# arihantb2/direct_lidar_odometry

Hardware: AMD Instinct MI355X
Metric: gicp_iterations_per_sec (higher is better)
Workload: dtype f64

## Files before the change

__graft_entry__.py:

```python
import os
import sys

ROOT = os.path.dirname(os.path.abspath(__file__))
if ROOT not in sys.path:
    sys.path.insert(0, ROOT)


def build() -> None:
    from direct_lidar_odometry_amd import build as b
    lib = b.build()
    assert os.path.exists(lib)
    import direct_lidar_odometry_amd
    from direct_lidar_odometry_amd import nano_gicp
    L = nano_gicp.load_library()
    missing = [s for s in nano_gicp.EXPORTS if not hasattr(L, s)]
    if missing:
        raise RuntimeError(f"libngicp_hip.so lacks {missing}")
    from oracle import oracle as orc
    orc.build(ref=os.path.isdir("/root/reference/include"))


def smoke() -> None:
    import numpy as np
    from direct_lidar_odometry_amd import build as b
    b.build()
    from direct_lidar_odometry_amd import clouds
    from direct_lidar_odometry_amd.nano_gicp import NanoGICP
    from oracle import oracle as orc

    w = clouds.scan_to_scan(10_000)
    g = NanoGICP(device=0)
    o = orc.OracleGICP()
    for e in (g, o):
        e.setMaxCorrespondenceDistance(1.0)
        e.setInputSource(w.source)
        e.setInputTarget(w.target)
    g.align()
    o.align()
    dt, dr = clouds.pose_error(g.getFinalTransformation(), o.getFinalTransformation())
    s = g.stats()
    print(f"smoke: HIP vs oracle pose diff {dt:.2e} m / {dr:.2e} rad; iterations {g.nr_iterations_ + 1} vs {o.nr_iterations + 1}; "
          f"align {s['align_ms']:.3f} ms; error vs ground truth {clouds.pose_error(g.getFinalTransformation(), w.gt)}")
    if not (dt <= 1e-4 and dr <= 1e-4 and g.nr_iterations_ == o.nr_iterations and g.converged_ == o.converged):
        raise AssertionError("HIP NanoGICP disagrees with the CPU oracle")


if __name__ == "__main__":
    build()
    if "--smoke" in sys.argv:
        smoke()
```

direct_lidar_odometry_amd/build.py:

```python
from __future__ import annotations

import os
import shutil
import subprocess
import sys

HERE = os.path.dirname(os.path.abspath(__file__))
CSRC = os.path.join(HERE, "csrc")
LIB = os.path.join(HERE, "libngicp_hip.so")
SOURCES = ["ngicp_api.hip", "ngicp_filters.hip"]
PUBLIC_HEADER = os.path.normpath(os.path.join(HERE, "..", "include", "ngicp.h"))
DEP_SUFFIXES = (".h", ".inc", ".hip")
FLAGS = ["--offload-arch=gfx950", "-O3", "-std=c++17", "-ffp-contract=off", "-fPIC", "-shared", "-Wall", "-Wno-unused-function"]


def hipcc() -> str:
    for cand in (os.environ.get("HIPCC"), shutil.which("hipcc"), "/opt/rocm/bin/hipcc"):
        if cand and os.path.exists(cand):
            return cand
    raise RuntimeError("hipcc not found")


def dependencies() -> list[str]:
    found = [os.path.join(d, f) for d, _, files in os.walk(CSRC) for f in files if f.endswith(DEP_SUFFIXES)]
    return sorted(found) + [PUBLIC_HEADER, os.path.abspath(__file__)]


def needs_build() -> bool:
    if not os.path.exists(LIB):
        return True
    t = os.path.getmtime(LIB)
    return any(os.path.getmtime(d) > t for d in dependencies())


def build(force: bool = False, verbose: bool = False, extra_flags: list[str] | None = None) -> str:
    if not force and not needs_build():
        return LIB
    tmp = f"{LIB}.{os.getpid()}.tmp"
    cmd = [hipcc(), *FLAGS, *(extra_flags or []), *[os.path.join(CSRC, s) for s in SOURCES], "-o", tmp]
    if verbose:
        print(" ".join(cmd), flush=True)
    res = subprocess.run(cmd, capture_output=True, text=True)
    if res.returncode != 0:
        sys.stderr.write(res.stdout + res.stderr)
        raise RuntimeError("hipcc failed")
    if verbose and res.stderr:
        sys.stderr.write(res.stderr)
    os.replace(tmp, LIB)
    return LIB


if __name__ == "__main__":
    print(build(force="--force" in sys.argv, verbose=True))
```

direct_lidar_odometry_amd/csrc/ngicp_align.h:

```cpp
#pragma once

namespace {

std::mutex& persist_mutex(int device) {
  static std::mutex m[64];
  return m[(unsigned)device % 64u];
}

route::Facts route_facts(const ngicp* h, route::Caller caller, int nblocks = 1) {
  route::Facts f;
  f.caller = caller;
  f.persist = h->persist;
  f.robust = h->robust_kind != NGICP_ROBUST_NONE;
  f.prior = h->prior_set;
  f.iterating = h->p.max_iter > 0;
  f.nblocks = nblocks;
  f.pass_slots = h->pass_slots;
  f.persist_slots = h->persist_slots;
  f.max_passes = max_passes(h->p);
  return f;
}
void refuse_for(const ngicp* h, route::Entry e) {
  const std::string why = route::entry_refusal(e, h->voxel_res > 0.0, h->robust_kind != NGICP_ROBUST_NONE, h->prior_set);
  if (!why.empty()) throw ArgError{NGICP_ERR_ARG, why};
}
void refuse_route(const ngicp* h, route::Caller caller, const char* entry) {
  const std::string why = route::refusal(route::switches(), h->sw, route_facts(h, caller), entry);
  if (!why.empty()) throw ArgError{NGICP_ERR_ARG, why};
}
route::Variant pass_variant(const ngicp* h, route::Caller caller, int nblocks) {
  return route::choose_route(route::switches(), h->sw, route_facts(h, caller, nblocks)).variant;
}
void fill_robust(const ngicp* h, int& kind, double& c, double& c2) {
  kind = h->robust_kind;
  c = h->robust_width;
  c2 = h->robust_width * h->robust_width;
}

void launch_pass(ngicp* h, const PassArgs& a, const route::Variant& v, int nblocks, hipStream_t s, hipEvent_t start = nullptr, hipEvent_t stop = nullptr) {
  using K = void (*)(PassArgs);
  const bool four = v.waves == 4;
  K kernel = nullptr;
  PassArgs b = a;
  unsigned grid = (unsigned)nblocks;
  switch (v.family) {
    case route::Family::Staged: {
      int need = kStGrowMax;
      if (h->p.max_corr_dist < 1e30) need = (int)std::ceil(h->p.max_corr_dist / (double)a.grid.h);
      b.stage_grow = std::max(1, std::min(kStGrowMax, need));
      kernel = four ? K(k_gicp_pass_st<4>) : K(k_gicp_pass_st<3>);
      break;
    }
    case route::Family::Queue:
      grid = (unsigned)std::min(nblocks, h->queue_slots[four]);
      kernel = four ? K(k_gicp_queue<2, 4>) : K(k_gicp_queue<2, 3>);
      break;
    case route::Family::Walks:
      if (v.fused) kernel = four ? K(k_gicp_pass<2, 4, true>) : K(k_gicp_pass<2, 3, true>);
      else if (v.robust) kernel = four ? K(k_gicp_pass<2, 4, false, true>) : K(k_gicp_pass<2, 3, false, true>);
      else kernel = four ? K(k_gicp_pass<2, 4>) : K(k_gicp_pass<2, 3>);
      break;
  }
  hipExtLaunchKernelGGL(kernel, dim3(grid), dim3(256), 0, s, start, stop, 0, b);
}

struct LoopCtx {
  PassArgs pa;
  SolveArgs sa;
  int nblocks;
};

void prepare_loop(ngicp* h, LoopCtx& c, bool own_buffers = true, bool with_target = true) {
  ensure_slot_ready(h, h->src, "source");
  if (with_target) ensure_slot_ready(h, h->tgt, "target");
  if (h->src_covs.n != h->src.dev->n) compute_covs(h, h->src, h->src_covs, "source");
  if (with_target && h->tgt_covs.n != h->tgt.dev->n) compute_covs(h, h->tgt, h->tgt_covs, "target");
  DeviceCloud& S = *h->src.dev;
  const size_t n = S.n;
  const int nblocks = std::max(1, (S.n_batches + 3) / 4);
  const int max_rows = max_trace_rows(h->p);
  if (own_buffers) {
    for (int i = 0; i < 2; ++i) {
      h->tpt[i].ensure(n * sizeof(float4));
      h->mahal[i].ensure(n * 6 * sizeof(double));
    }
    h->partials.ensure((size_t)kNumSlots * nblocks * sizeof(double));
    h->grp_order.ensure((size_t)nblocks * sizeof(int));
    h->grp_order_alt.ensure((size_t)nblocks * sizeof(int));
    h->grp_cost.ensure((size_t)nblocks * sizeof(int));
    {
      const long ring = (long)max_rows + 1;
      h->state.ensure(sizeof(LmState) + (ring <= kMaxPersistPasses ? (size_t)ring * kViewWords * sizeof(int) : 0));
    }
    if (h->trace.ensure_grew((size_t)max_rows * kTraceCols * sizeof(double))) h->trace_rows_dev = 0;
    h->sums.ensure(kPartialStride * sizeof(double));
    h->batch_far.ensure((size_t)S.n_batches + 16);
    h->gen_lines.ensure((size_t)kGenLines * kGenStride * sizeof(int));
  }

  PassArgs& a = c.pa;
  fill_robust(h, a.robust_kind, a.robust_c, a.robust_c2);
  a.qpts = S.qpts.as<float4>();
  a.batches = S.batches.as<int2>();
  a.batch_boxes = S.batch_boxes.as<float>();
  int* const order_buf[2] = {own_buffers ? h->grp_order.as<int>() : nullptr, own_buffers ? h->grp_order_alt.as<int>() : nullptr};
  int* const ctl = own_buffers ? h->order_flag.as<int>() : nullptr;
  int* const order_flag[2] = {ctl, ctl ? ctl + 3 : nullptr};
  a.grp_order = order_buf[h->order_sel];
  a.grp_cost = own_buffers ? h->grp_cost.as<int>() : nullptr;
  a.n_batches = S.n_batches;
  a.cov_src = covs_for(h, h->src_covs, h->src.dev);
  a.n_src = (int)n;
  if (with_target) {
    DeviceCloud& T = *h->tgt.dev;
    a.tgt = T.pts();
    a.tgt3 = T.xyz3();
    a.tgtp = T.xyzp();
    a.tgt_cell_start = T.cells();
    a.tgt_cell_box = (h->sw.cell_boxes && T.has_boxes) ? T.cell_box.as<unsigned int>() + kCellPad : nullptr;
    a.cov_tgt = covs_for(h, h->tgt_covs, h->tgt.dev);
    a.grid = T.grid;
  } else {
    a.tgt = nullptr;
    a.tgt3 = nullptr;
    a.tgtp = nullptr;
    a.tgt_cell_start = nullptr;
    a.tgt_cell_box = nullptr;
    a.cov_tgt = nullptr;
    a.grid = Grid{};
  }
  for (int i = 0; i < 2; ++i) {
    a.tpt[i] = own_buffers ? h->tpt[i].as<float4>() : nullptr;
    a.mahal[i] = own_buffers ? h->mahal[i].as<double>() : nullptr;
  }
  a.gate_sq = h->p.max_corr_dist * h->p.max_corr_dist;
  {
    float f = (float)a.gate_sq;
    if ((double)f < a.gate_sq) f = std::nextafter(f, std::numeric_limits<float>::infinity());
    a.gate_sq_f = f;
  }
  a.batch_far = own_buffers ? h->batch_far.as<unsigned char>() : nullptr;
  a.st = own_buffers ? h->state.as<LmState>() : nullptr;
  a.partials = own_buffers ? h->partials.as<double>() : nullptr;
  a.mode = 3;
  a.dbg_stamps = nullptr;
  a.dbg_qstats = nullptr;
  a.dbg_span = nullptr;
  a.order_valid = order_flag[h->order_sel];
  a.t_first = nullptr;
  a.fused = 0;
  a.persist = 0;
  a.first_pass = 0;
  a.max_passes = 0;
  a.ticket = ctl ? ctl + 1 : nullptr;
  a.gen = own_buffers ? h->gen_lines.as<int>() : nullptr;
  {
    int need = kStageMaxGrow;
    if (with_target && h->p.max_corr_dist < 1e30) need = (int)std::ceil(h->p.max_corr_dist / (double)a.grid.h);
    a.stage_grow = h->sw.stage_grow <= 0 ? 0 : std::max(1, std::min(std::min(kStageMaxGrow, h->sw.stage_grow), need));
  }

  SolveArgs& s = c.sa;
  s.st = a.st;
  s.cfg.max_iterations = h->p.max_iter;
  s.cfg.lm_max_iterations = h->p.lm_max_iter;
  s.cfg.optimizer = h->p.optimizer;
  s.cfg.rot_eps = h->p.rot_eps;
  s.cfg.trans_eps = h->p.trans_eps;
  s.cfg.lm_init_lambda_factor = h->p.lm_init_lambda_factor;
  s.partials = a.partials;
  s.nblocks = nblocks;
  s.grp_order = order_buf[h->order_sel];
  s.grp_cost = a.grp_cost;
  s.trace = own_buffers ? h->trace.as<double>() : nullptr;
  s.max_trace_rows = max_rows;
  s.mode = 0;
  s.sums_out = nullptr;
  s.dbg_stamps = nullptr;
  s.progress_host = nullptr;
  s.final_host = nullptr;
  s.order_valid = order_flag[h->order_sel];
  s.t_first = nullptr;
  s.persist = 0;
  s.pass_honours_word = 0;
  s.serial_step = h->sw.serial_step;
  s.pass_ticks = nullptr;
  s.prior = h->prior_set ? h->prior_dev.as<double>() : nullptr;
  s.st_out = nullptr;
  s.nrows = 0;
  a.crow_in = nullptr;
  a.crow_out = nullptr;
  a.cluster_ticket = nullptr;
  a.done_flag = nullptr;
  c.nblocks = nblocks;
  if (!own_buffers) return;
  h->stats.lanes_per_query = 2;
  h->stats.voxel_size = a.grid.h;
  h->stats.grid_dims[0] = a.grid.nx;
  h->stats.grid_dims[1] = a.grid.ny;
  h->stats.grid_dims[2] = a.grid.nz;
}

void init_state_from_pose(LmState& st, const Pose& x0) {
  std::memset(&st, 0, sizeof(st));
  st.hot.x0 = x0;
  st.hot.xi = x0;
  pose_identity(st.hot.delta);
  for (int r = 0; r < 3; ++r) {
    for (int c = 0; c < 3; ++c) st.xi_f[r * 4 + c] = (float)x0.R[r * 3 + c];
    st.xi_f[r * 4 + 3] = (float)x0.t[r];
  }
  std::memcpy(&st.view[kViewXi], &st.hot.xi, sizeof(Pose));
  std::memcpy(&st.view[kViewXiF], st.xi_f, sizeof(st.xi_f));
  static_assert(sizeof(Pose) == 24 * sizeof(int) && kViewXiF == 24 && sizeof(LmState::xi_f) == 12 * sizeof(int), "LmState::view layout");
  st.hot.lambda = -1.0;
  st.hot.nu = 2.0;
// ... 245 lines not shown
    if (le != hipSuccess) {
      (void)hipGetLastError();
      launched_ok = false;
    }
  } else {
    hipLaunchKernelGGL((k_gicp_persist<2, 3>), dim3((unsigned)grid), dim3(256), 0, h->stream, pa);
  }
  bool ok = false;
  while (launched_ok) {
    const int prog = __atomic_load_n(h->h_progress, __ATOMIC_ACQUIRE);
    if (prog & kProgressDone) {
      ok = true;
      break;
    }
    if ((++al.spins & 0x3fff) == 0) {
      if (hipStreamQuery(h->stream) == hipSuccess) {
        ok = (__atomic_load_n(h->h_progress, __ATOMIC_ACQUIRE) & kProgressDone) != 0;
        break;
      }
      if (now_ms() - al.t_loop > 30000.0) throw ArgError{NGICP_ERR_HIP, "the registration loop did not finish within 30 s"};
    }
    if (h->host_wait) sched_yield(); else __builtin_ia32_pause();
  }
  if (ok) {
    al.st.hot = *h->pin_final;
    al.loop_ms = (float)((double)(al.st.hot.t_done - al.st.hot.t_first) * 1e-5);
    if (al.st.hot.passes >= 3 && c.nblocks <= kMaxOrderGroups) h->order_sel = sel ^ 1;
    return true;
  }
  std::fprintf(stderr, launched_ok ? "ngicp: the persistent registration kernel gave up waiting; falling back to one launch per pass\n"
                                   : "ngicp: the persistent registration kernel could not be launched; falling back to one launch per pass\n");
  h->persist = 0;
  HIP_TRY(hipMemsetAsync(h->order_flag.p, 0, 4 * sizeof(int), h->stream));
  HIP_TRY(hipMemcpyAsync(h->state.p, &h->pin_state[0], sizeof(LmState), hipMemcpyHostToDevice, h->stream));
  *h->h_progress = 0;
  return false;
}

void sum_tick_pass_times(ngicp* h, const LmHot& hot) {
  ngicp_stats& s = h->stats;
  const long timed = std::min<long>(hot.passes, kMaxTickPasses);
  int counted = 0;
  if (max_trace_rows(h->p) <= kMaxTickPasses) {
    for (long i = 0; i < timed; ++i) {
      const unsigned long long from = i == 0 ? hot.t_first : h->pin_ticks[2 * (i - 1) + 1], to = h->pin_ticks[2 * i];
      if (to > from) {
        s.pass_ms_total += (double)(to - from) * 1e-5;
        ++counted;
      }
    }
  }
  s.passes_timed = counted;
  if (std::getenv("NGICP_DEBUG_TICKS")) {
    std::fprintf(stderr, "persistent kernel, pass / step us:");
    for (long i = 0; i < timed; ++i) {
      const unsigned long long from = i == 0 ? hot.t_first : h->pin_ticks[2 * (i - 1) + 1];
      std::fprintf(stderr, " %.1f/%.1f", (double)(h->pin_ticks[2 * i] - from) * 1e-2, (double)(h->pin_ticks[2 * i + 1] - h->pin_ticks[2 * i]) * 1e-2);
    }
    std::fprintf(stderr, "\n");
  }
}

constexpr size_t kHeadCrowBytes = (size_t)kSolveRowSubsets * kNumSlots * sizeof(double);
void head_begin(ngicp* h) {
  h->state_alt.ensure(sizeof(LmState));
  h->head_ws.ensure(64 + 128 + 2 * kHeadCrowBytes);
  HIP_TRY(hipMemsetAsync(h->head_ws.p, 0, 64 + 128 + 2 * kHeadCrowBytes, h->stream));
}
void launch_head(ngicp* h, const LoopCtx& c, long launched, hipEvent_t start, hipEvent_t stop) {
  unsigned char* const ws = h->head_ws.as<unsigned char>();
  int* const ctl = h->order_flag.as<int>();
  LmState* const state[2] = {h->state.as<LmState>(), h->state_alt.as<LmState>()};
  double* const crow[2] = {reinterpret_cast<double*>(ws + 192), reinterpret_cast<double*>(ws + 192 + kHeadCrowBytes)};
  int* const order[2] = {h->grp_order.as<int>(), h->grp_order_alt.as<int>()};
  int* const flag[2] = {ctl, ctl + 3};
  const int par = (int)(launched & 1);
  PassArgs pa = c.pa;
  pa.st = state[par];
  pa.crow_in = crow[par];
  pa.crow_out = crow[par ^ 1];
  pa.cluster_ticket = reinterpret_cast<int*>(ws + 64);
  pa.done_flag = reinterpret_cast<int*>(ws);
  pa.grp_order = order[par];
  pa.order_valid = flag[par];
  pa.sa = c.sa;
  pa.sa.st = state[par];
  pa.sa.st_out = state[par ^ 1];
  pa.sa.partials = crow[par];
  pa.sa.nrows = kSolveRowSubsets;
  pa.sa.grp_order = order[par ^ 1];
  pa.sa.order_valid = flag[par ^ 1];
  hipExtLaunchKernelGGL((k_gicp_head<2, 3>), dim3((unsigned)c.nblocks + 1), dim3(256), 0, h->stream, start, stop, 0, pa);
}

void launch_persist_one(ngicp* h, const LoopCtx& c, long launched, hipEvent_t start, hipEvent_t stop) {
  PassArgs pa = c.pa;
  pa.fused = 1;
  pa.persist = route::switches().persist_one;
  pa.first_pass = (int)launched;
  pa.max_passes = 1;
  pa.sa = c.sa;
  pa.sa.persist = 1;
  HIP_TRY(hipMemsetAsync(pa.ticket, 0, sizeof(int), h->stream));
  HIP_TRY(hipMemsetAsync(h->gen_lines.p, 0, (size_t)kGenLines * kGenStride * sizeof(int), h->stream));
  hipExtLaunchKernelGGL((k_gicp_persist<2, 3>), dim3((unsigned)std::min(c.nblocks, h->persist_slots)), dim3(256), 0, h->stream, start, stop, 0, pa);
}

void do_align(ngicp* h, const float guess[16], float* aligned, size_t out_stride) {
  refuse_route(h, route::Caller::Align, "ngicp_align");
  Alignment al;
  reset_results(h);
  LoopCtx c;
  prepare_loop(h, c);
  if (!(h->order_src == h->src.dev.get() && h->order_groups == c.sa.nblocks)) HIP_TRY(hipMemsetAsync(h->order_flag.p, 0, 4 * sizeof(int), h->stream));
  route::Facts f = route_facts(h, route::Caller::Align, c.nblocks);
  f.xcd_installed = install_xcd_order(h, c);
  set_pass_mode(h, c.pa);
  allow_k4_only_passes(h, c, f);
  if (const char* dbg = std::getenv("NGICP_DEBUG_MODE")) c.pa.mode |= (std::atoi(dbg) & (8 | 16));
  begin_alignment(h, al, guess, c.sa, c.pa.t_first);
  const DebugDumps dbg = debug_begin(h, c);
  f.dump_stamps = dbg.stamp_path != nullptr;
  f.dump_span = dbg.span_path != nullptr;
  f.dump_qstats = dbg.qstat_path != nullptr;
  f.dump_solve = c.sa.dbg_stamps != nullptr;
  const route::Choice pick = route::choose_route(route::switches(), h->sw, f);
  const long max_p = f.max_passes;
  const bool persist_done = pick.route == route::Route::Persist && align_persistent(h, c, al, max_p);
  switch (persist_done ? route::Route::Persist : pick.fallback) {
    case route::Route::Persist:
      break;
    case route::Route::Head:
      head_begin(h);
      feed_alignment(h, al, max_p + 1, [&](long i, hipEvent_t start, hipEvent_t stop) { launch_head(h, c, i, start, stop); });
      if ((al.st.hot.passes + 1) & 1) HIP_TRY(hipMemcpyAsync(h->state.p, h->state_alt.p, sizeof(LmState), hipMemcpyDeviceToDevice, h->stream));
      break;
    case route::Route::PersistOne:
      feed_alignment(h, al, max_p, [&](long i, hipEvent_t start, hipEvent_t stop) { launch_persist_one(h, c, i, start, stop); });
      break;
    case route::Route::Fused:
      c.pa.fused = 1;
      c.pa.sa = c.sa;
      HIP_TRY(hipMemsetAsync(c.pa.ticket, 0, sizeof(int), h->stream));
      [[fallthrough]];
    case route::Route::Default:
    case route::Route::Staged:
    case route::Route::Queue: {
      const long stamp_launch = route::switches().debug_solve_launch;
      feed_alignment(h, al, max_p, [&](long i, hipEvent_t start, hipEvent_t stop) {
        launch_pass(h, c.pa, pick.variant, c.nblocks, h->stream, start, stop);
        if (!route::row(pick.fallback).own_solver) return;
        SolveArgs sa = c.sa;
        if (stamp_launch > 1 && i + 1 != stamp_launch) sa.dbg_stamps = nullptr;
        hipLaunchKernelGGL(k_lm_solve, dim3(1), dim3(kSolveThreads), 0, h->stream, sa);
      });
      break;
    }
  }
  HIP_TRY(hipGetLastError());
  debug_end(h, c, dbg);
  end_alignment(h, al, aligned, out_stride, !persist_done);
  ngicp_stats& s = h->stats;
  h->order_src = h->src.dev.get();
  h->order_groups = c.sa.nblocks;
  s.staged_fraction = al.st.hot.search_passes > 0 ? al.st.hot.staged_total / ((double)al.st.hot.search_passes * (double)h->src.dev->n) : 0.0;
  if (al.st.hot.search_passes > 1) h->prev_staged_fraction = s.staged_fraction;
  if (persist_done && h->profiling) sum_tick_pass_times(h, al.st.hot);
}

struct VoxelCtx {
  VoxelPassArgs pa;
  SolveArgs sa;
  int nblocks;
};

template <class F>
void with_voxel_variant(int nbr, bool robust, F&& f) {
  auto with_k = [&](auto k) { robust ? f(k, std::true_type{}) : f(k, std::false_type{}); };
  switch (nbr) {
    case NGICP_VOX_DIRECT1: with_k(std::integral_constant<int, 1>{}); break;
    case NGICP_VOX_DIRECT7: with_k(std::integral_constant<int, 7>{}); break;
    case NGICP_VOX_DIRECT27: with_k(std::integral_constant<int, 27>{}); break;
    default: throw ArgError{NGICP_ERR_STATE, "voxelized GICP: unknown neighbourhood"};
  }
}

void launch_voxel_pass(ngicp* h, const VoxelCtx& c, hipEvent_t start = nullptr, hipEvent_t stop = nullptr) {
  const dim3 grid((unsigned)c.nblocks), block(kVoxBlock);
  with_voxel_variant(c.pa.nbr, c.pa.robust_kind != NGICP_ROBUST_NONE, [&](auto k, auto robust) {
    constexpr int K = decltype(k)::value;
    constexpr bool R = decltype(robust)::value;
    if constexpr (K == 1) hipExtLaunchKernelGGL(k_vgicp_pass<R>, grid, block, 0, h->stream, start, stop, 0, c.pa);
    else hipExtLaunchKernelGGL((k_vgicp_pass_n<K, R>), grid, block, 0, h->stream, start, stop, 0, c.pa);
  });
}

void fill_voxel_shared(ngicp* h, VoxelPassArgs& a, const VoxelMapView& m) {
  DeviceCloud& S = *h->src.dev;
  a.src = S.pts();
  a.cov_src = covs_for(h, h->src_covs, h->src.dev);
  a.n_src = (int)S.n;
  a.table = m.table;
  a.mask = m.mask;
  a.rec = m.rec;
  a.n_vox = (int)m.n_vox;
  a.inv_res = 1.0f / (float)h->voxel_res;
  a.nbr = h->voxel_nbr;
  a.slot_stride = (int)S.n;
  a.mode = 3;
  a.t_first = nullptr;
  fill_robust(h, a.robust_kind, a.robust_c, a.robust_c2);
}

void prepare_voxel_loop(ngicp* h, VoxelCtx& v) {
  LoopCtx c;
  prepare_loop(h, c, true, !rolling_active(h));
  const VoxelMapView vm = ensure_voxel_map(h);
  DeviceCloud& S = *h->src.dev;
  const size_t n = S.n;
  const int nblocks = std::max(1, (int)((n + kVoxBlock - 1) / kVoxBlock));
  h->partials.ensure((size_t)kNumSlots * nblocks * sizeof(double));
  const size_t K = (size_t)h->voxel_nbr;
  for (int i = 0; i < 2; ++i) {
    h->vox_corr[i].ensure(K * n * sizeof(int));
    if (K > 1) h->vox_mahal[i].ensure(K * n * 6 * sizeof(double));
  }
  VoxelPassArgs& a = v.pa;
  fill_voxel_shared(h, a, vm);
  for (int i = 0; i < 2; ++i) {
    a.corr[i] = h->vox_corr[i].as<int>();
    a.mahal[i] = K > 1 ? h->vox_mahal[i].as<double>() : h->mahal[i].as<double>();
  }
  a.st = h->state.as<LmState>();
  a.partials = h->partials.as<double>();
  v.sa = c.sa;
  v.sa.partials = a.partials;
  v.sa.nblocks = nblocks;
  v.sa.grp_order = nullptr;
  v.sa.grp_cost = nullptr;
  v.sa.order_valid = nullptr;
  v.nblocks = nblocks;
}

void do_align_voxel(ngicp* h, const float guess[16], float* aligned, size_t out_stride) {
  Alignment al;
  reset_results(h);
  VoxelCtx c;
  prepare_voxel_loop(h, c);
  c.pa.mode = (h->p.optimizer == NGICP_OPT_GAUSS_NEWTON) ? 2 : 3;
  begin_alignment(h, al, guess, c.sa, c.pa.t_first);
  feed_alignment(h, al, max_passes(h->p), [&](long, hipEvent_t start, hipEvent_t stop) {
    launch_voxel_pass(h, c, start, stop);
    hipLaunchKernelGGL(k_lm_solve, dim3(1), dim3(kSolveThreads), 0, h->stream, c.sa);
  });
  HIP_TRY(hipGetLastError());
  end_alignment(h, al, aligned, out_stride);
  h->stats.staged_fraction = 0.0;
}

struct HookCtx {
  bool vox;
  LoopCtx c;
  VoxelCtx vc;
  route::Variant variant;
};
void prepare_hook(ngicp* h, HookCtx& k) {
  k.vox = h->voxel_res > 0.0;
  if (k.vox) {
    prepare_voxel_loop(h, k.vc);
    return;
  }
  refuse_route(h, route::Caller::Hook, "linearize / compute_error");
  prepare_loop(h, k.c);
  k.variant = pass_variant(h, route::Caller::Hook, k.c.nblocks);
}
void launch_hook(ngicp* h, HookCtx& k, int pass_mode, int solve_mode) {
  if (k.vox) {
    k.vc.pa.mode = pass_mode;
    launch_voxel_pass(h, k.vc);
  } else {
    k.c.pa.mode = pass_mode;
    launch_pass(h, k.c.pa, k.variant, k.c.nblocks, h->stream);
  }
  SolveArgs sa = k.vox ? k.vc.sa : k.c.sa;
  sa.mode = solve_mode;
  hipLaunchKernelGGL(k_lm_solve, dim3(1), dim3(kSolveThreads), 0, h->stream, sa);
}

size_t round_up(size_t v, size_t a) { return (v + a - 1) / a * a; }

void ensure_batch_pinned(ngicp* h) {
  BatchWs& w = h->batch;
  if (!w.pin_recs) HIP_TRY(hipHostMalloc(reinterpret_cast<void**>(&w.pin_recs), (size_t)kBatchMaxLanes * (sizeof(LmState) + sizeof(PassArgs) + sizeof(SolveArgs)), hipHostMallocDefault));
  if (!w.pin_progress) HIP_TRY(hipHostMalloc(reinterpret_cast<void**>(&w.pin_progress), (size_t)kBatchMaxLanes * BatchWs::kProgressStride * sizeof(int), hipHostMallocDefault));
  if (!w.pin_final) HIP_TRY(hipHostMalloc(reinterpret_cast<void**>(&w.pin_final), (size_t)kBatchMaxLanes * sizeof(LmHot), hipHostMallocDefault));
}

template <class LaunchPass>
void feed_batch(ngicp* h, int B, BatchLaunch& bl, long max_passes, std::vector<LmHot>& result, LaunchPass&& launch_pass_batch) {
  BatchWs& w = h->batch;
  const int depth = h->sw.chunk;
  const double t_loop = now_ms();
  unsigned long spins = 0;
  bool idle_seen = false;
  auto look_at_stream = [&]() -> bool {
    const hipError_t q = hipStreamQuery(h->stream);
    if (q == hipErrorNotReady) {
      (void)hipGetLastError();
    } else if (q != hipSuccess) {
      throw HipError{q, "hipStreamQuery(h->stream)", __FILE__, __LINE__};
    }
    if (now_ms() - t_loop > 30000.0) throw ArgError{NGICP_ERR_HIP, "the batched registration loop did not finish within 30 s"};
    return q == hipSuccess;
  };
  auto relax = [&]() {
    if (idle_seen) throw ArgError{NGICP_ERR_HIP, "the batched registration loop: the stream is idle but a lane has not reported"};
    if ((++spins & (h->host_wait ? 0xff : 0xfff)) == 0 && look_at_stream()) {
      idle_seen = true;
      return;
    }
    if (h->host_wait) sched_yield(); else __builtin_ia32_pause();
  };
  long launched = 0;
  int n_live = B;
  std::vector<int> live((size_t)B);
  for (int g = 0; g < B; ++g) live[(size_t)g] = g;
  for (;;) {
    long min_prog = std::numeric_limits<long>::max();
    int keep_n = 0;
    for (int i = 0; i < n_live; ++i) {
      const int g = live[(size_t)i];
      const int prog = __atomic_load_n(w.pin_progress + (size_t)g * BatchWs::kProgressStride, __ATOMIC_ACQUIRE);
      if (prog & kProgressDone) {
        result[(size_t)g] = w.pin_final[g];
        continue;
      }
      live[(size_t)keep_n++] = g;
      min_prog = std::min(min_prog, (long)(prog & kProgressMask));
    }
    n_live = keep_n;
    if (n_live == 0) break;
    if (launched >= max_passes || launched - min_prog >= depth) {
      relax();
      continue;
    }
    idle_seen = false;
    for (int i = 0; i < n_live; ++i) bl.lane[i] = live[(size_t)i];
    launch_pass_batch(bl, n_live);
    hipLaunchKernelGGL(k_lm_solve_batch, dim3((unsigned)n_live), dim3(kSolveThreads), 0, h->stream, bl);
    ++launched;
  }
}

void return_batch_results(ngicp* h, const std::vector<LmHot>& result, size_t trace_stride, float* T_out, int* converged, int* nr_iterations, double* hessians) {
  BatchWs& w = h->batch;
  for (size_t g = 0; g < result.size(); ++g) {
    store_result(result[g], T_out + g * 16, converged ? converged + g : nullptr, nr_iterations ? nr_iterations + g : nullptr, hessians ? hessians + g * 36 : nullptr);
    w.trace_rows.push_back((size_t)result[g].n_trace);
  }
  w.lanes = (int)result.size();
  w.trace_stride = trace_stride;
}

struct BatchRecs {
  int B;
  size_t off_pass, off_solve, bytes, part_stride, trace_stride;
  LmState* st_host;
  unsigned char* pass_host;
  SolveArgs* sa_host;
  unsigned char* dev;
};

BatchRecs batch_begin(ngicp* h, int B, size_t pass_size, int nblocks) {
  BatchWs& w = h->batch;
  BatchRecs r;
  r.B = B;
  r.off_pass = (size_t)B * sizeof(LmState);
  r.off_solve = r.off_pass + round_up((size_t)B * pass_size, 16);
  r.bytes = r.off_solve + (size_t)B * sizeof(SolveArgs);
  r.part_stride = (size_t)nblocks * kNumSlots * sizeof(double);
  r.trace_stride = (size_t)max_trace_rows(h->p) * kTraceCols;
  w.lanes = 0;
  w.trace_rows.clear();
  ensure_batch_pinned(h);
  w.recs.ensure(r.bytes);
  w.partials.ensure((size_t)B * r.part_stride);
  w.trace.ensure((size_t)B * r.trace_stride * sizeof(double));
  r.st_host = reinterpret_cast<LmState*>(w.pin_recs);
  r.pass_host = w.pin_recs + r.off_pass;
  r.sa_host = reinterpret_cast<SolveArgs*>(w.pin_recs + r.off_solve);
  r.dev = w.recs.as<unsigned char>();
  return r;
}

SolveArgs batch_lane(ngicp* h, const BatchRecs& r, int g, const float* guesses, const SolveArgs& shared) {
  BatchWs& w = h->batch;
  init_state_from_pose(r.st_host[g], pose_from_colmajor(guesses + (size_t)g * 16));
  if (h->p.max_iter <= 0) r.st_host[g].hot.done = 1;
  SolveArgs sa = shared;
  sa.st = reinterpret_cast<LmState*>(r.dev) + g;
  sa.partials = reinterpret_cast<double*>(w.partials.as<unsigned char>() + (size_t)g * r.part_stride);
  sa.trace = w.trace.as<double>() + (size_t)g * r.trace_stride;
  sa.progress_host = w.pin_progress + (size_t)g * BatchWs::kProgressStride;
  sa.final_host = w.pin_final + g;
  sa.t_first = nullptr;
  *sa.progress_host = 0;
  return sa;
}

template <class LaunchPass>
void run_batch(ngicp* h, const BatchRecs& r, float* T_out, int* converged, int* nr_iterations, double* hessians, LaunchPass&& launch_pass_batch) {
  std::vector<LmHot> result((size_t)r.B);
  if (h->p.max_iter <= 0) {
    for (int g = 0; g < r.B; ++g) result[(size_t)g] = r.st_host[g].hot;
  } else {
    HIP_TRY(hipMemcpyAsync(r.dev, h->batch.pin_recs, r.bytes, hipMemcpyHostToDevice, h->stream));
    BatchLaunch bl;
    bl.pass = r.dev + r.off_pass;
    bl.solve = reinterpret_cast<const SolveArgs*>(r.dev + r.off_solve);
    for (int i = 0; i < kBatchMaxLanes; ++i) bl.lane[i] = 0;
    feed_batch(h, r.B, bl, max_passes(h->p), result, launch_pass_batch);
    HIP_TRY(hipGetLastError());
  }
  return_batch_results(h, result, r.trace_stride, T_out, converged, nr_iterations, hessians);
}

void do_align_batch(ngicp* h, int B, const float* guesses, float* T_out, int* converged, int* nr_iterations, double* hessians) {
  BatchWs& w = h->batch;
  LoopCtx c;
  prepare_loop(h, c, false);
  set_pass_mode(h, c.pa);

  const size_t n = h->src.dev->n;
  const int nblocks = c.nblocks, n_batches = c.pa.n_batches;
  const size_t tpt_stride = round_up(n * sizeof(float4), 256), mahal_stride = round_up(n * 6 * sizeof(double), 256);
  const size_t ord_stride = round_up((size_t)nblocks * sizeof(int), 256), far_stride = round_up((size_t)n_batches + 16, 256);
  const bool order_described = w.order_src == h->src.dev.get() && w.order_groups == nblocks && w.order_lanes >= B;
  const int lanes_before = w.order_lanes;
  w.order_src = nullptr;
  w.order_lanes = 0;
  const BatchRecs r = batch_begin(h, B, sizeof(PassArgs), nblocks);
  w.tpt.ensure((size_t)B * 2 * tpt_stride);
  w.mahal.ensure((size_t)B * 2 * mahal_stride);
  bool order_kept = order_described;
  if (w.order.ensure_grew((size_t)B * ord_stride)) order_kept = false;
  w.cost.ensure((size_t)B * ord_stride);
  if (w.flags.ensure_grew((size_t)kBatchMaxLanes * 4 * sizeof(int))) order_kept = false;
  if (w.far.ensure_grew((size_t)B * far_stride)) HIP_TRY(hipMemsetAsync(w.far.p, 0, w.far.cap, h->stream));
  if (!order_kept) HIP_TRY(hipMemsetAsync(w.flags.p, 0, (size_t)kBatchMaxLanes * 4 * sizeof(int), h->stream));

  PassArgs* const pa_host = reinterpret_cast<PassArgs*>(r.pass_host);
  for (int g = 0; g < B; ++g) {
    SolveArgs sa = batch_lane(h, r, g, guesses, c.sa);
    PassArgs pa = c.pa;
    pa.st = sa.st;
    for (int i = 0; i < 2; ++i) {
      pa.tpt[i] = reinterpret_cast<float4*>(w.tpt.as<unsigned char>() + ((size_t)g * 2 + i) * tpt_stride);
      pa.mahal[i] = reinterpret_cast<double*>(w.mahal.as<unsigned char>() + ((size_t)g * 2 + i) * mahal_stride);
    }
    pa.partials = const_cast<double*>(sa.partials);
    pa.grp_order = reinterpret_cast<int*>(w.order.as<unsigned char>() + (size_t)g * ord_stride);
    pa.grp_cost = reinterpret_cast<int*>(w.cost.as<unsigned char>() + (size_t)g * ord_stride);
    pa.batch_far = w.far.as<unsigned char>() + (size_t)g * far_stride;
    pa.order_valid = w.flags.as<int>() + (size_t)g * 4;
    pa.ticket = w.flags.as<int>() + (size_t)g * 4 + 1;
    pa.t_first = nullptr;
    sa.grp_order = const_cast<int*>(pa.grp_order);
    sa.grp_cost = pa.grp_cost;
    sa.order_valid = const_cast<int*>(pa.order_valid);
    pa.sa = sa;
    pa_host[g] = pa;
    r.sa_host[g] = sa;
  }
  run_batch(h, r, T_out, converged, nr_iterations, hessians, [&](const BatchLaunch& l, int n_live) {
    const bool four = (long)nblocks * n_live > 2L * h->pass_slots;
    if (four)
      hipLaunchKernelGGL((k_gicp_pass_batch<2, 4>), dim3((unsigned)nblocks, (unsigned)n_live), dim3(256), 0, h->stream, l);
    else
      hipLaunchKernelGGL((k_gicp_pass_batch<2, 3>), dim3((unsigned)nblocks, (unsigned)n_live), dim3(256), 0, h->stream, l);
  });
  w.order_src = h->src.dev.get();
  w.order_groups = nblocks;
  w.order_lanes = std::max(order_kept ? lanes_before : 0, B);
}

void do_align_voxel_batch(ngicp* h, int B, const float* guesses, float* T_out, int* converged, int* nr_iterations, double* hessians) {
  static_assert(sizeof(VoxelPassArgs) <= sizeof(PassArgs), "the pinned record block is sized for PassArgs records");
  BatchWs& w = h->batch;
  LoopCtx c;
  prepare_loop(h, c, false, !rolling_active(h));
  const VoxelMapView vm = ensure_voxel_map(h);
  const size_t n = h->src.dev->n, K = (size_t)h->voxel_nbr;
  const int nblocks = std::max(1, (int)((n + kVoxBlock - 1) / kVoxBlock));
  const size_t corr_stride = round_up(K * n * sizeof(int), 256), mahal_stride = round_up(K * n * 6 * sizeof(double), 256);
  const BatchRecs r = batch_begin(h, B, sizeof(VoxelPassArgs), nblocks);
  w.vox_corr.ensure((size_t)B * 2 * corr_stride);
  w.vox_mahal.ensure((size_t)B * 2 * mahal_stride);
  VoxelPassArgs shared;
  fill_voxel_shared(h, shared, vm);
  shared.mode = (h->p.optimizer == NGICP_OPT_GAUSS_NEWTON) ? 2 : 3;
  SolveArgs solve = c.sa;
  solve.nblocks = nblocks;
  solve.grp_order = nullptr;
  solve.grp_cost = nullptr;
  solve.order_valid = nullptr;
  VoxelPassArgs* const pa_host = reinterpret_cast<VoxelPassArgs*>(r.pass_host);
  for (int g = 0; g < B; ++g) {
    const SolveArgs sa = batch_lane(h, r, g, guesses, solve);
    VoxelPassArgs pa = shared;
    pa.st = sa.st;
    for (int i = 0; i < 2; ++i) {
      pa.corr[i] = reinterpret_cast<int*>(w.vox_corr.as<unsigned char>() + ((size_t)g * 2 + i) * corr_stride);
      pa.mahal[i] = reinterpret_cast<double*>(w.vox_mahal.as<unsigned char>() + ((size_t)g * 2 + i) * mahal_stride);
    }
    pa.partials = const_cast<double*>(sa.partials);
    pa_host[g] = pa;
    r.sa_host[g] = sa;
  }
  run_batch(h, r, T_out, converged, nr_iterations, hessians, [&](const BatchLaunch& l, int n_live) {
    const dim3 grid((unsigned)nblocks, (unsigned)n_live), block(kVoxBlock);
    with_voxel_variant((int)K, false, [&](auto k, auto) { hipLaunchKernelGGL(k_vgicp_pass_batch<decltype(k)::value>, grid, block, 0, h->stream, l); });
  });
}

}
```

direct_lidar_odometry_amd/csrc/ngicp_api.hip:

```cpp
#include "../../include/ngicp.h"

#include <hip/hip_runtime.h>
#include <hip/hip_ext.h>

#include <algorithm>
#include <atomic>
#include <chrono>
#include <cmath>
#include <cstdio>
#include <cstdlib>
#include <cstring>
#include <limits>
#include <memory>
#include <mutex>
#include <sched.h>
#include <string>
#include <vector>

#include "ngicp_route.h"
#include "ngicp_pass.h"
#include "ngicp_cloudops.h"
#include "ngicp_filters.h"
#include "ngicp_query.h"
#include "ngicp_range.h"
// ... 1328 lines not shown
    hipLaunchKernelGGL(k_scan2_tile_sums, dim3(1), dim3(kScanBlock), 0, h->stream, h->tile_sums.as<unsigned long long>(), ntiles);
    hipLaunchKernelGGL(k_scan64_apply, dim3(ntiles), dim3(kScanBlock), 0, h->stream, h->rad_counts.as<int>(), n, h->tile_sums.as<unsigned long long>(),
                       h->rad_offsets.as<unsigned long long>());
    static_assert(sizeof(size_t) == sizeof(unsigned long long), "offsets are copied as they are");
    int n_long = 0;
    HIP_TRY(hipMemcpyAsync(offsets, h->rad_offsets.p, (nq + 1) * sizeof(size_t), hipMemcpyDeviceToHost, h->stream));
    HIP_TRY(hipMemcpyAsync(&n_long, n_long_dev, sizeof(int), hipMemcpyDeviceToHost, h->stream));
    HIP_TRY(hipStreamSynchronize(h->stream));
    const size_t tot = offsets[nq];
    if (n_long > 0 && C.n > ((size_t)1 << 30)) throw ArgError{NGICP_ERR_ARG, "segments beyond 2^30 points are not sorted by this engine"};
    if (tot > ((size_t)1 << 40) / sizeof(unsigned long long)) throw HipError{hipErrorOutOfMemory, "radius search result buffer", __FILE__, __LINE__};
    if (tot) {
      h->rad_keys.ensure(tot * sizeof(unsigned long long));
      hipLaunchKernelGGL(k_radius_walk<true>, wgrid, dim3(kRadBlock), 0, h->stream, C.pts(), C.cells(), C.grid, h->queries.as<float4>(), n, rf, reach,
                         (int*)nullptr, h->rad_offsets.as<unsigned long long>(), h->rad_keys.as<unsigned long long>(), (int*)nullptr, (int*)nullptr);
      hipLaunchKernelGGL(k_seg_sort_short, dim3((unsigned)((nq + kSegBlock / 64 - 1) / (kSegBlock / 64))), dim3(kSegBlock), 0, h->stream,
                         h->rad_offsets.as<unsigned long long>(), n, h->rad_keys.as<unsigned long long>());
      if (n_long > 0)
        hipLaunchKernelGGL(k_seg_sort_long, dim3((unsigned)n_long), dim3(kSegLongBlock), 0, h->stream, h->rad_offsets.as<unsigned long long>(), n_long_dev + 1,
                           h->rad_keys.as<unsigned long long>());
    }
    HIP_TRY(hipEventRecord(h->ev_q_b, h->stream));
    HIP_TRY(hipStreamSynchronize(h->stream));
    HIP_TRY(hipGetLastError());
    query_timing_done(h);
    h->rad_total = tot;
    h->rad_valid = true;
    *total = tot;
  });
}

int ngicp_radius_fetch(ngicp_t* h, int* idx, float* sqd, size_t capacity) {
  return guarded(h, [&] {
    if (!idx || !sqd) throw ArgError{NGICP_ERR_ARG, "null output"};
    if (!h->rad_valid) throw ArgError{NGICP_ERR_STATE, "no radius search to fetch"};
    const size_t tot = h->rad_total;
    if (capacity < tot) throw ArgError{NGICP_ERR_ARG, "capacity is smaller than the search's total"};
    if (tot == 0) return;
    h->knn_idx.ensure(tot * sizeof(int));
    h->knn_d2.ensure(tot * sizeof(float));
    hipLaunchKernelGGL(k_radius_unpack, dim3((unsigned)std::min<size_t>((tot + 255) / 256, 4096)), dim3(256), 0, h->stream, h->rad_keys.as<unsigned long long>(), tot,
                       h->knn_idx.as<int>(), h->knn_d2.as<float>());
    HIP_TRY(hipMemcpyAsync(idx, h->knn_idx.p, tot * sizeof(int), hipMemcpyDeviceToHost, h->stream));
    HIP_TRY(hipMemcpyAsync(sqd, h->knn_d2.p, tot * sizeof(float), hipMemcpyDeviceToHost, h->stream));
    HIP_TRY(hipStreamSynchronize(h->stream));
    HIP_TRY(hipGetLastError());
  });
}

int ngicp_fitness_score(ngicp_t* h, const float T_colmajor[16], double max_range, double* score, size_t* n_inliers) {
  return guarded(h, [&] {
    if (!score) throw ArgError{NGICP_ERR_ARG, "null output"};
    DeviceCloud& S = query_cloud(h, 0);
    DeviceCloud& T = query_cloud(h, 1);
    const int n = (int)S.n;
    const int nb = (n + kKnnPairs - 1) / kKnnPairs;
    h->fit_T.ensure(16 * sizeof(float));
    h->fit_part.ensure((size_t)nb * sizeof(double2));
    h->fit_out.ensure(sizeof(double2));
    HIP_TRY(hipMemcpyAsync(h->fit_T.p, T_colmajor ? T_colmajor : h->final_T, 16 * sizeof(float), hipMemcpyHostToDevice, h->stream));
    HIP_TRY(hipEventRecord(h->ev_q_a, h->stream));
    hipLaunchKernelGGL(k_fitness, dim3((unsigned)nb, 1u), dim3(kKnnBlock), 0, h->stream, S.pts(), n, h->fit_T.as<float>(), T.pts(), T.cells(), T.grid, max_range,
                       h->fit_part.as<double2>());
    hipLaunchKernelGGL(k_fitness_final, dim3(1), dim3(kFitnessFinalBlock), 0, h->stream, h->fit_part.as<double2>(), nb, h->fit_out.as<double2>());
    HIP_TRY(hipEventRecord(h->ev_q_b, h->stream));
    double2 r;
    HIP_TRY(hipMemcpyAsync(&r, h->fit_out.p, sizeof(r), hipMemcpyDeviceToHost, h->stream));
    HIP_TRY(hipStreamSynchronize(h->stream));
    HIP_TRY(hipGetLastError());
    query_timing_done(h);
    const size_t cnt = (size_t)r.y;
    *score = cnt ? r.x / r.y : std::numeric_limits<double>::max();
    if (n_inliers) *n_inliers = cnt;
  });
}

int ngicp_range_select(ngicp_t* h, int which, size_t rank, float* value, size_t* n_points) {
  return guarded(h, [&] { range_select_impl(h, which, rank, false, value, n_points); });
}

int ngicp_range_median(ngicp_t* h, int which, float* value, size_t* n_points) {
  return guarded(h, [&] { range_select_impl(h, which, 0, true, value, n_points); });
}

int ngicp_get_lm_trace(ngicp_t* h, double* rows, size_t max_rows, size_t* n_rows) {
  return guarded(h, [&] {
    if (h->trace_host.empty() && h->trace_rows_dev) {
      h->trace_host.resize(h->trace_rows_dev * kTraceCols);
      HIP_TRY(hipMemcpyAsync(h->trace_host.data(), h->trace.p, h->trace_host.size() * sizeof(double), hipMemcpyDeviceToHost, h->stream));
      HIP_TRY(hipStreamSynchronize(h->stream));
    }
    const size_t n = h->trace_host.size() / kTraceCols;
    if (n_rows) *n_rows = n;
    if (rows) std::memcpy(rows, h->trace_host.data(), std::min(n, max_rows) * kTraceCols * sizeof(double));
  });
}

int ngicp_get_stats(ngicp_t* h, ngicp_stats* out) {
  if (!h || !out) return NGICP_ERR_ARG;
  if (h->cov_timing_pending) {
    float ms = 0.f;
    if (hipEventSynchronize(h->ev_cov_b) == hipSuccess && hipEventElapsedTime(&ms, h->ev_cov_a, h->ev_cov_b) == hipSuccess) h->stats.covariance_ms = ms;
    h->cov_timing_pending = false;
  }
  h->stats.device_allocs = g_device_allocs.load(std::memory_order_relaxed);
  *out = h->stats;
  return NGICP_OK;
}
int ngicp_set_host_wait(ngicp_t* h, int mode) {
  if (!h || (mode != 0 && mode != 1)) return NGICP_ERR_ARG;
  h->host_wait = mode;
  return NGICP_OK;
}
int ngicp_set_profiling(ngicp_t* h, int on) {
  return guarded(h, [&] {
    h->profiling = on != 0;
    h->prof_stride = on > 1 ? on : 1;
    if (h->profiling && h->prof_events.empty()) {
      h->prof_events.resize(2 * 1024);
      for (auto& e : h->prof_events) HIP_TRY(hipEventCreate(&e));
    }
  });
}

int ngicp_sharded_begin(ngicp_t* h, const float guess[16]) {
  return guarded(h, [&] {
    refuse_for(h, route::Entry::ShardedBegin);
    h->shard_ctx.reset(new LoopCtx);
    LoopCtx& c = *h->shard_ctx;
    prepare_loop(h, c);
    set_pass_mode(h, c.pa);
    allow_k4_only_passes(h, c, route_facts(h, route::Caller::Sharded));
    upload_initial_state(h, guess ? guess : kIdentity16);
    HIP_TRY(hipStreamSynchronize(h->stream));
    for (int i = 0; i < kShardSlots; ++i) h->h_shard_done[i] = 0;
    h->shard_steps = 0;
    h->sharded_active = true;
    h->hook_valid = 0;
  });
}

int ngicp_sharded_pass(ngicp_t* h, double* sums32_dev, void* stream_or_null) {
  return guarded(h, [&] {
    refuse_for(h, route::Entry::ShardedPass);
    if (!h->sharded_active || !h->shard_ctx) throw ArgError{NGICP_ERR_STATE, "ngicp_sharded_begin not called"};
    if (!sums32_dev) throw ArgError{NGICP_ERR_ARG, "null sums buffer"};
    hipStream_t s = stream_or_null ? (hipStream_t)stream_or_null : h->stream;
    LoopCtx& c = *h->shard_ctx;
    launch_pass(h, c.pa, pass_variant(h, route::Caller::Sharded, c.nblocks), c.nblocks, s);
    SolveArgs sa = c.sa;
    sa.mode = 3;
    sa.sums_out = sums32_dev;
    sa.grp_order = nullptr;
    hipLaunchKernelGGL(k_lm_solve, dim3(1), dim3(kSolveThreads), 0, s, sa);
    HIP_TRY(hipGetLastError());
  });
}

int ngicp_sharded_step(ngicp_t* h, const double* sums32_dev, void* stream_or_null, int* done) {
  return guarded(h, [&] {
    refuse_for(h, route::Entry::ShardedStep);
    if (!h->sharded_active || !h->shard_ctx) throw ArgError{NGICP_ERR_STATE, "ngicp_sharded_begin not called"};
    if (!sums32_dev) throw ArgError{NGICP_ERR_ARG, "null sums buffer"};
    hipStream_t s = stream_or_null ? (hipStream_t)stream_or_null : h->stream;
    LoopCtx& c = *h->shard_ctx;
    SolveArgs sa = c.sa;
    sa.mode = 0;
    sa.partials = sums32_dev;
    sa.nblocks = 1;
    sa.grp_order = nullptr;
    hipLaunchKernelGGL(k_lm_solve, dim3(1), dim3(kSolveThreads), 0, s, sa);
    h->shard_stream = s;
    const long k = h->shard_steps++;
    const int slot = (int)(k % kShardSlots);
    LmState* dst = h->state.as<LmState>();
    HIP_TRY(hipMemcpyAsync(&h->h_shard_done[slot], &dst->hot.done, sizeof(int), hipMemcpyDeviceToHost, s));
    HIP_TRY(hipEventRecord(h->ev_shard[slot], s));
    HIP_TRY(hipGetLastError());
    int d = 0;
    if (k >= kShardLag) {
      const int old = (int)((k - kShardLag) % kShardSlots);
      HIP_TRY(hipEventSynchronize(h->ev_shard[old]));
      d = h->h_shard_done[old];
    }
    if (done) *done = d;
  });
}

int ngicp_sharded_finish(ngicp_t* h, float T_out[16], int* converged, int* nr_iterations, double final_hessian[36]) {
  return guarded(h, [&] {
    refuse_for(h, route::Entry::ShardedFinish);
    if (!h->sharded_active) throw ArgError{NGICP_ERR_STATE, "ngicp_sharded_begin not called"};
    hipStream_t s = h->shard_stream ? h->shard_stream : h->stream;
    HIP_TRY(hipMemcpyAsync(&h->pin_state[1], h->state.p, sizeof(LmState), hipMemcpyDeviceToHost, s));
    HIP_TRY(hipStreamSynchronize(s));
    store_result(h->pin_state[1].hot, h->final_T, &h->converged, &h->nr_iterations, h->final_hessian);
    copy_results_out(h, T_out, converged, nr_iterations, final_hessian);
    h->stats.passes = h->pin_state[1].hot.passes;
    h->stats.search_passes = h->pin_state[1].hot.search_passes;
    h->stats.lm_trials = h->pin_state[1].hot.n_trace;
    h->sharded_active = false;
    h->shard_ctx.reset();
    h->shard_stream = nullptr;
  });
}

int ngicp_covs_shard_begin(ngicp_t* h, int which, double** covs6_dev, size_t* n_points) {
  return guarded(h, [&] {
    refuse_for(h, route::Entry::CovsShardBegin);
    if ((which != 0 && which != 1) || !covs6_dev || !n_points) throw ArgError{NGICP_ERR_ARG, "bad argument"};
    Slot& slot = which ? h->tgt : h->src;
    ensure_slot_ready(h, slot, which ? "target" : "source");
    CovSet& cs = h->shard_covs[which];
    cs.data = acquire_buf(h, h->device, slot.dev->n * 6 * sizeof(double));
    cs.n = slot.dev->n;
    cs.order = slot.dev;
    HIP_TRY(hipStreamSynchronize(h->stream));
    *covs6_dev = cs.data->as<double>();
    *n_points = cs.n;
  });
}
int ngicp_covs_shard_compute(ngicp_t* h, int which, size_t lo, size_t hi, void* stream_or_null) {
  return guarded(h, [&] {
    refuse_for(h, route::Entry::CovsShardCompute);
    if (which != 0 && which != 1) throw ArgError{NGICP_ERR_ARG, "bad argument"};
    CovSet& cs = h->shard_covs[which];
    Slot& slot = which ? h->tgt : h->src;
    if (!cs.data || cs.order.get() != slot.dev.get()) throw ArgError{NGICP_ERR_STATE, "ngicp_covs_shard_begin not called for this cloud"};
    if (lo > hi || hi > cs.n) throw ArgError{NGICP_ERR_ARG, "block outside the cloud"};
    launch_cov_range(h, *slot.dev, cs.data->as<double>(), lo, hi, stream_or_null ? (hipStream_t)stream_or_null : h->stream);
    HIP_TRY(hipGetLastError());
  });
}
int ngicp_covs_shard_commit(ngicp_t* h, int which) {
  return guarded(h, [&] {
    refuse_for(h, route::Entry::CovsShardCommit);
    if (which != 0 && which != 1) throw ArgError{NGICP_ERR_ARG, "bad argument"};
    CovSet& cs = h->shard_covs[which];
    Slot& slot = which ? h->tgt : h->src;
    if (!cs.data || cs.order.get() != slot.dev.get()) throw ArgError{NGICP_ERR_STATE, "ngicp_covs_shard_begin not called for this cloud"};
    (which ? h->tgt_covs : h->src_covs) = cs;
    cs.clear();
  });
}

int ngicp_keyframe_add(ngicp_t* h, ngicp_t* from, int* id_out) {
  if (!from) return NGICP_ERR_ARG;
  return guarded(h, [&] {
    if (h->device != from->device) throw ArgError{NGICP_ERR_ARG, "keyframe_add across devices is not supported"};
    ensure_slot_ready(from, from->src, "source");
    if (from->src_covs.n != from->src.dev->n) compute_covs(from, from->src, from->src_covs, "source");
    (void)covs_for(from, from->src_covs, from->src.dev);
    HIP_TRY(hipStreamSynchronize(from->stream));
    h->keyframes.push_back({from->src.dev, from->src_covs.data});
    if (id_out) *id_out = (int)h->keyframes.size() - 1;
  });
}

int ngicp_keyframe_add_transformed(ngicp_t* h, ngicp_t* from, const float T_colmajor[16], int* id_out) {
  if (!from) return NGICP_ERR_ARG;
  return guarded(h, [&] {
    if (!T_colmajor) throw ArgError{NGICP_ERR_ARG, "null transform"};
    if (h->device != from->device) throw ArgError{NGICP_ERR_ARG, "keyframe_add across devices is not supported"};
    ensure_slot_ready(from, from->src, "source");
    DeviceCloud& S = *from->src.dev;
    const size_t n = S.n;
    from->tfinal.ensure(16 * sizeof(float));
    HIP_TRY(hipMemcpyAsync(from->tfinal.p, T_colmajor, 16 * sizeof(float), hipMemcpyHostToDevice, from->stream));
    from->unsorted.ensure(n * sizeof(float4));
    const int bbox_blocks = pick_blocks(n, 1024, 512);
    from->bbox.ensure((size_t)bbox_blocks * 8 * sizeof(float));
    hipLaunchKernelGGL(k_transform_to_unsorted, dim3(bbox_blocks), dim3(256), 0, from->stream, S.pts(), (int)n, from->tfinal.as<float>(), from->unsorted.as<float4>(),
                       from->bbox.as<float>());
    std::vector<float> bb((size_t)bbox_blocks * 8);
    HIP_TRY(hipMemcpyAsync(bb.data(), from->bbox.p, bb.size() * sizeof(float), hipMemcpyDeviceToHost, from->stream));
    HIP_TRY(hipStreamSynchronize(from->stream));
    float mn[3] = {3.0e38f, 3.0e38f, 3.0e38f}, mx[3] = {-3.0e38f, -3.0e38f, -3.0e38f};
    for (int b = 0; b < bbox_blocks; ++b)
      for (int d = 0; d < 3; ++d) {
        mn[d] = std::min(mn[d], bb[(size_t)b * 8 + d]);
        mx[d] = std::max(mx[d], bb[(size_t)b * 8 + 3 + d]);
      }
    for (int d = 0; d < 3; ++d)
      if (!std::isfinite(mn[d]) || !std::isfinite(mx[d]) || mn[d] > mx[d]) throw ArgError{NGICP_ERR_ARG, "transform produced non-finite coordinates"};
    Slot tmp;
    tmp.present = true;
    tmp.n = n;
    tmp.dev = index_unsorted(from, n, mn, mx);
    CovSet cs;
    compute_covs(from, tmp, cs, "keyframe");
    HIP_TRY(hipStreamSynchronize(from->stream));
    h->keyframes.push_back({tmp.dev, cs.data});
    if (id_out) *id_out = (int)h->keyframes.size() - 1;
  });
}

int ngicp_keyframe_add_transformed_filtered(ngicp_t* h, ngicp_t* from, const float T_colmajor[16], float leaf, int* id_out) {
  if (!from) return NGICP_ERR_ARG;
  if (!(leaf > 0.f)) return ngicp_keyframe_add_transformed(h, from, T_colmajor, id_out);
  return guarded(h, [&] {
    if (!T_colmajor) throw ArgError{NGICP_ERR_ARG, "null transform"};
    if (h->device != from->device) throw ArgError{NGICP_ERR_ARG, "keyframe_add across devices is not supported"};
    ensure_slot_ready(from, from->src, "source");
    DeviceCloud& S = *from->src.dev;
    const size_t n = S.n;
    from->tfinal.ensure(16 * sizeof(float));
    HIP_TRY(hipMemcpyAsync(from->tfinal.p, T_colmajor, 16 * sizeof(float), hipMemcpyHostToDevice, from->stream));
    from->xyzi.ensure(n * sizeof(float4));
    hipLaunchKernelGGL(k_transform_sorted_to_original4, dim3((unsigned)((n + 255) / 256)), dim3(256), 0, from->stream, S.pts(), (int)n, from->tfinal.as<float>(),
                       from->xyzi.as<float4>());
    from->filt_out = nullptr;
    from->filt_n = 0;
    char err[256] = {0};
    const float4* out = nullptr;
    int m = 0;
    if (ngk_filter_cloud(from->stream, &from->fws, from->xyzi.as<float4>(), (int)n, 0, 0.f, leaf, &out, &m, err, sizeof(err))) throw ArgError{NGICP_ERR_HIP, err};
    if (m <= 0) throw ArgError{NGICP_ERR_ARG, "the voxel filter left no points"};
    from->unsorted.ensure((size_t)m * sizeof(float4));
    const int bbox_blocks = pick_blocks((size_t)m, 1024, 512);
    from->bbox.ensure((size_t)bbox_blocks * 8 * sizeof(float));
    hipLaunchKernelGGL(k_xyzi_to_unsorted, dim3(bbox_blocks), dim3(256), 0, from->stream, out, m, from->unsorted.as<float4>(), from->bbox.as<float>());
    std::vector<float> bb((size_t)bbox_blocks * 8);
    HIP_TRY(hipMemcpyAsync(bb.data(), from->bbox.p, bb.size() * sizeof(float), hipMemcpyDeviceToHost, from->stream));
    HIP_TRY(hipStreamSynchronize(from->stream));
// ... 544 lines not shown
```

direct_lidar_odometry_amd/csrc/ngicp_batch.h:

```cpp
#pragma once
#include "ngicp_pass.h"
#include "ngicp_query.h"

namespace ngk {

constexpr int kBatchMaxLanes = 64;

struct BatchLaunch {
  const void* pass;
  const SolveArgs* solve;
  int lane[kBatchMaxLanes];
};
typedef const BatchLaunch __attribute__((address_space(4))) KernelBatchLaunch;

#define NG_STAMP(k) \
  do {              \
  } while (0)
template <int G, int WPS>
__device__ __forceinline__ void batch_group_body(KernelPassArgs& a, const int group, WaveStage* stage_all, double (*lds)[kNumSlots]) {
  constexpr bool FUSED = false;
  constexpr int B = 64 / G;
  constexpr int kWin = WPS >= 4 ? 12 : 16, kSideStep = WPS >= 4 ? 8 : 16;
  static_assert(kWin <= kSortedPad && B == kBatchQueries, "see k_gicp_pass");
  const bool do_lin = (a.mode & 2);
  Grid g;
  g.ox = a.grid.ox; g.oy = a.grid.oy; g.oz = a.grid.oz;
  g.h = a.grid.h; g.inv_h = a.grid.inv_h;
  g.nx = a.grid.nx; g.ny = a.grid.ny; g.nz = a.grid.nz;
  g.ncells = a.grid.ncells;
  g.slack = a.grid.slack;
  typedef const double __attribute__((address_space(4))) * ViewPtrD;
  typedef const float __attribute__((address_space(4))) * ViewPtrF;
  KernelStatePtr st4 = (KernelStatePtr)(unsigned long long)a.st;
  const int have_lin = st4->hot.have_lin;
  const int cur = st4->hot.cur & 1, nxt = cur ^ 1;
  ViewPtrD vx = (ViewPtrD)&st4->hot.xi;
  ViewPtrF vf = (ViewPtrF)st4->xi_f;
  double R[9], t[3];
  float Tf[12];
#pragma unroll
  for (int i = 0; i < 9; ++i) R[i] = vx[i];
#pragma unroll
  for (int i = 0; i < 3; ++i) t[i] = vx[9 + i];
#pragma unroll
  for (int i = 0; i < 12; ++i) Tf[i] = vf[i];
  const bool do_err = (a.mode & 1) && have_lin;
  const float4* __restrict__ tpt_old = a.tpt[cur];
  const double* __restrict__ mahal_old = a.mahal[cur];
  float4* __restrict__ tpt_new = a.tpt[nxt];
  double* __restrict__ mahal_new = a.mahal[nxt];
  double wave_total = 0.0;
  unsigned int ncand = 0, nvalid = 0, nstaged = 0;
  const int lane = threadIdx.x & 63, wave = __builtin_amdgcn_readfirstlane((int)(threadIdx.x >> 6));
  const int sub = lane % G, grp = lane / G;
  WaveStage& S = stage_all[wave];
  const unsigned long long t_start = a.grp_cost ? __builtin_amdgcn_s_memtime() : 0ull;
#define NG_HAVE_LIN have_lin
#include "ngicp_pass_group.inc"
#undef NG_HAVE_LIN
}
#undef NG_STAMP

template <int G, int WPS>
__global__ void __launch_bounds__(256, WPS) k_gicp_pass_batch(BatchLaunch bl) {
  __shared__ WaveStage stage[4];
  __shared__ double lds[4][kNumSlots];
  KernelBatchLaunch* kb = (KernelBatchLaunch*)__builtin_amdgcn_kernarg_segment_ptr();
  const int lane_id = kb->lane[blockIdx.y];
  KernelPassArgs* ka = (KernelPassArgs*)(unsigned long long)(reinterpret_cast<const PassArgs*>(kb->pass) + lane_id);
  typedef const int __attribute__((address_space(4))) * ConstIntPtr;
  const int done_now = ((KernelStatePtr)(unsigned long long)ka->st)->hot.done;
  const int order_is_valid = *(ConstIntPtr)(unsigned long long)ka->order_valid;
  const int order_entry = ((ConstIntPtr)(unsigned long long)ka->grp_order)[blockIdx.x];
  asm volatile("" ::"s"(done_now), "s"(order_is_valid), "s"(order_entry));
  if (done_now) return;
  const int group = order_is_valid ? order_entry : (int)blockIdx.x;
  batch_group_body<G, WPS>(*ka, group, stage, lds);
}

__global__ void __launch_bounds__(kSolveThreads) k_lm_solve_batch(BatchLaunch bl) {
  __shared__ SolveShared<kSolveThreads> sh;
  KernelBatchLaunch* kb = (KernelBatchLaunch*)__builtin_amdgcn_kernarg_segment_ptr();
  const int lane_id = kb->lane[blockIdx.x];
  static_assert(sizeof(SolveArgs) % 4 == 0, "SolveArgs is copied as dwords");
  constexpr int kWords = (int)(sizeof(SolveArgs) / 4);
  typedef const int __attribute__((address_space(4))) * ConstIntPtr;
  ConstIntPtr src = (ConstIntPtr)(unsigned long long)(kb->solve + lane_id);
  int w[kWords];
#pragma unroll
  for (int i = 0; i < kWords; ++i) w[i] = src[i];
  SolveArgs a;
  __builtin_memcpy(&a, w, sizeof(a));
  lm_solve_body<kSolveThreads, false>(a, sh);
}

}
```

direct_lidar_odometry_amd/csrc/ngicp_lm.h:

```cpp
#pragma once
#include <stddef.h>

#include "ngicp_math.h"
#include "ngicp_terms.h"

namespace ngk {

struct LmConfig {
  int max_iterations;
  int lm_max_iterations;
  int optimizer;
  double rot_eps, trans_eps;
  double lm_init_lambda_factor;
};

struct LmHot {
  Pose x0;
  Pose xi;
  Pose delta;
  double H[36];
  double b[6];
  double y0;
  double d[6];
  double lambda, nu;
  double cand_total;
  double valid_total;
  double staged_total;
  int iter;
  int trial;
  int have_lin;
  int cur;
  int done;
  int converged;
  int nr_iterations;
  int lm_failed;
  int n_trace;
  int passes;
  int pending;
  double final_H[36];
  unsigned long long t_first, t_done;
  float lin_f[12];
  int lin_unneeded;
  int search_passes;
};
constexpr int kViewXi = 0;
constexpr int kViewXiF = 24;
constexpr int kViewDone = 36, kViewCur = 37, kViewHaveLin = 38;
struct LmState {
  LmHot hot;
  float xi_f[12];
  alignas(512) int view[128];
};
constexpr int kViewWords = 128;
constexpr int kGenLines = 256, kGenStride = 32;
static_assert(sizeof(LmState) % 512 == 0 && offsetof(LmState, view) % 512 == 0, "ring entries are 512-byte aligned");

struct PassPose {
  double R[9], t[3];
  float Tf[12];
  int have_lin, cur;
};
typedef const LmState __attribute__((address_space(4))) * KernelStatePtr;
template <class S>
__device__ __forceinline__ void load_pose(S st, PassPose& p) {
  p.have_lin = st->hot.have_lin;
  p.cur = st->hot.cur;
#pragma unroll
  for (int i = 0; i < 9; ++i) p.R[i] = st->hot.xi.R[i];
#pragma unroll
  for (int i = 0; i < 3; ++i) p.t[i] = st->hot.xi.t[i];
#pragma unroll
  for (int i = 0; i < 12; ++i) p.Tf[i] = st->xi_f[i];
}

struct SolveArgs {
  LmState* st;
  LmConfig cfg;
  const double* partials;
  int nblocks;
  double* trace;
  int max_trace_rows;
  int mode;
  double* sums_out;
  int* grp_order;
  const int* grp_cost;
  unsigned long long* dbg_stamps;
  int* progress_host;
  LmHot* final_host;
  int* order_valid;
  const unsigned long long* t_first;
  LmState* st_out;
  int nrows;
  int persist;
  int pass_honours_word;
  int serial_step;
  unsigned long long* pass_ticks;
  const double* prior;
};

static_assert(offsetof(SolveArgs, pass_ticks) == offsetof(SolveArgs, pass_honours_word) + 8, "serial_step takes no room of its own");

__host__ __device__ __forceinline__ int tri21(int r, int c) { return r * 6 - (r * (r - 1)) / 2 + (c - r); }

constexpr int kMaxOrderGroups = 4096;
constexpr int kSolveThreads = 512;
constexpr int kSolveRowSubsets = 32;
constexpr int kProgressDone = 1 << 30, kProgressMask = kProgressDone - 1;

__device__ __forceinline__ bool is_converged_dev(const Pose& d, double rot_eps, double trans_eps) {
  double rmax = 0.0, tmax = 0.0;
#pragma unroll
  for (int r = 0; r < 3; ++r) {
#pragma unroll
    for (int c = 0; c < 3; ++c) rmax = fmax(rmax, 1.0 / rot_eps * fabs(d.R[r * 3 + c] - (r == c ? 1.0 : 0.0)));
    tmax = fmax(tmax, 1.0 / trans_eps * fabs(d.t[r]));
  }
  return fmax(rmax, tmax) < 1;
}

__device__ __forceinline__ double lm_gain_den(const double* d, const double* b, const double lambda) {
  double den = 0.0;
#pragma unroll
  for (int i = 0; i < 6; ++i) den += d[i] * (lambda * d[i] - b[i]);
  return den;
}
__device__ __forceinline__ double lm_step_norm2(const double* d) {
  double dn = 0.0;
#pragma unroll
  for (int i = 0; i < 6; ++i) dn += d[i] * d[i];
  return dn;
}
__device__ __forceinline__ double lm_lambda_accepted(const double lambda, const double rho) {
  const double q = 2 * rho - 1;
  return lambda * fmax(1.0 / 3.0, 1 - q * q * q);
}

__device__ __forceinline__ void make_trial(LmHot& L, double lambda_add) {
  double A[36], rhs[6];
#pragma unroll
  for (int i = 0; i < 36; ++i) A[i] = L.H[i];
#pragma unroll
  for (int i = 0; i < 6; ++i) {
    A[i * 6 + i] += lambda_add;
    rhs[i] = -L.b[i];
  }
  ldlt6_solve(A, rhs, L.d);
  pose_identity(L.delta);
  so3_exp_matrix(L.d, L.delta.R);
  L.delta.t[0] = L.d[3];
  L.delta.t[1] = L.d[4];
  L.delta.t[2] = L.d[5];
  pose_mul(L.delta, L.x0, L.xi);
}

__device__ __forceinline__ void set_lin_unneeded(LmHot& L, const LmConfig& cfg) {
  L.lin_unneeded = (is_converged_dev(L.delta, cfg.rot_eps, cfg.trans_eps) || L.iter + 1 >= cfg.max_iterations) ? 1 : 0;
}

__device__ __forceinline__ void adopt_new(LmHot& L, const double* sums) {
#pragma unroll
  for (int r = 0; r < 6; ++r)
#pragma unroll
    for (int c = r; c < 6; ++c) L.H[r * 6 + c] = L.H[c * 6 + r] = sums[tri21(r, c)];
#pragma unroll
  for (int i = 0; i < 6; ++i) L.b[i] = sums[21 + i];
  L.y0 = sums[27];
  L.cur ^= 1;
  L.have_lin = 1;
#pragma unroll
  for (int r = 0; r < 3; ++r) {
#pragma unroll
    for (int c = 0; c < 3; ++c) L.lin_f[r * 4 + c] = (float)L.xi.R[r * 3 + c];
    L.lin_f[r * 4 + 3] = (float)L.xi.t[r];
  }
}

__device__ __forceinline__ bool lm_advance(LmHot& L, const LmConfig& cfg, const double* sums, double* trace, int max_trace_rows) {
  const double yi = sums[28];
  L.passes += 1;
  L.cand_total += sums[29];
  L.valid_total += sums[30];
  L.staged_total += sums[31];

  if (cfg.optimizer == 0) {
    adopt_new(L, sums);
    L.nr_iterations = L.iter;
    make_trial(L, 0.0);
    L.x0 = L.xi;
    L.converged = is_converged_dev(L.delta, cfg.rot_eps, cfg.trans_eps) ? 1 : 0;
    L.iter += 1;
    if (L.converged || L.iter >= cfg.max_iterations) L.done = 1;
    return true;
  }

  if (!L.have_lin) {
    adopt_new(L, sums);
    L.nr_iterations = 0;
    if (L.lambda < 0.0) {
      double m = 0.0;
#pragma unroll
      for (int i = 0; i < 6; ++i) m = fmax(m, fabs(L.H[i * 6 + i]));
      L.lambda = cfg.lm_init_lambda_factor * m;
    }
    L.nu = 2.0;
    L.trial = 0;
    if (cfg.lm_max_iterations <= 0) {
      L.lm_failed = 1;
      L.done = 1;
      return false;
    }
    make_trial(L, L.lambda);
    set_lin_unneeded(L, cfg);
    return false;
  }

  const double den = lm_gain_den(L.d, L.b, L.lambda), dn = lm_step_norm2(L.d);
  const double rho = (L.y0 - yi) / den;
  const bool rejected = rho < 0;
  if (trace && L.n_trace < max_trace_rows) {
    double* row = trace + (size_t)L.n_trace * kTraceCols;
    row[0] = L.iter; row[1] = L.trial; row[2] = L.y0; row[3] = yi;
    row[4] = rho; row[5] = L.lambda; row[6] = sqrt(dn); row[7] = rejected ? 0.0 : 1.0;
    L.n_trace += 1;
  }
  if (rejected) {
    if (is_converged_dev(L.delta, cfg.rot_eps, cfg.trans_eps)) {
      L.converged = 1;
      L.done = 1;
      return false;
    }
    L.lambda = L.nu * L.lambda;
    L.nu = 2 * L.nu;
    L.trial += 1;
    if (L.trial >= cfg.lm_max_iterations) {
      L.lm_failed = 1;
      L.converged = 0;
      L.done = 1;
      return false;
    }
    make_trial(L, L.lambda);
    set_lin_unneeded(L, cfg);
    return false;
  }
  return true;
}

__device__ __forceinline__ void lm_step(LmHot& L, const LmConfig& cfg, const double* sums, double* trace, int max_trace_rows, const bool searched = true) {
  const bool gn = cfg.optimizer == 0;
  L.search_passes += searched ? 1 : 0;
  const bool accepted = lm_advance(L, cfg, sums, trace, max_trace_rows);
  if (accepted) {
#pragma unroll
    for (int i = 0; i < 36; ++i) L.final_H[i] = L.H[i];
    if (!gn) {
// ... 253 lines not shown
```

direct_lidar_odometry_amd/csrc/ngicp_pass.h:

```cpp
#pragma once
#include <type_traits>

#include "../../include/ngicp.h"
#include "ngicp_knn.h"
#include "ngicp_terms.h"
#include "ngicp_lm.h"
#include "ngicp_search.h"
#include "ngicp_solve.h"

namespace ngk {

struct PassArgs {
  const float4* qpts;
  const int2* batches;
  const float* batch_boxes;
  const int* grp_order;
  int* grp_cost;
  int n_batches;
  const double* cov_src;
  int n_src;
  const float4* tgt;
  const float4* tgtp;
  const Xyz* tgt3;
  const int* tgt_cell_start;
  const unsigned int* tgt_cell_box;
  const double* cov_tgt;
  Grid grid;
  float4* tpt[2];
  double* mahal[2];
  double gate_sq;
  float gate_sq_f;
  unsigned char* batch_far;
  LmState* st;
  double* partials;
  int mode;
  int stage_grow;
  unsigned long long* dbg_stamps;
  int4* dbg_qstats;
  unsigned long long* dbg_span;
  const int* order_valid;
  unsigned long long* t_first;
  int fused;
  int* ticket;
  const double* crow_in;
  double* crow_out;
  int* cluster_ticket;
  int* done_flag;
  int persist;
  int first_pass;
  int max_passes;
  int* gen;
  SolveArgs sa;
  int robust_kind;
  double robust_c, robust_c2;
};

constexpr int kStampStride = 24;
#define NG_STAMP(k)                                                                                   \
  do {                                                                                                \
    if (a.dbg_stamps && lane == 0) a.dbg_stamps[(size_t)(blockIdx.x * 4 + wave) * kStampStride + (k)] = __builtin_amdgcn_s_memtime(); \
  } while (0)

template <int G, int WPS = NGICP_PASS_WAVES, bool FUSED = false, bool ROBUST = false>
__global__ void __launch_bounds__(256, WPS) k_gicp_pass(PassArgs a) {
  constexpr int B = 64 / G;
  constexpr int kWin = WPS >= 4 ? 12 : 16, kSideStep = WPS >= 4 ? 8 : 16;
  static_assert(kWin <= kSortedPad, "walk windows may overhang the array by at most the sentinel frame");
  static_assert(B == kBatchQueries, "query batches are built for 32 queries (2 lanes per query)");
  __shared__ double lds[4][kNumSlots];
  struct Nothing {};
  union PassShared {
    WaveStage stage[4];
    typename std::conditional<FUSED, SolveShared<256>, Nothing>::type sv;
  };
  __shared__ PassShared shm;
  __shared__ int last_block;
  WaveStage* stage_all = shm.stage;
  const LmState* __restrict__ st = a.st;
  typedef const int __attribute__((address_space(4))) * ConstIntPtr;
  const int done_now = st->hot.done, have_lin_now = st->hot.have_lin;
  const int cur = st->hot.cur, nxt = cur ^ 1;
  const int lin_unneeded_now = st->hot.lin_unneeded;
  const int order_is_valid = *(ConstIntPtr)(unsigned long long)a.order_valid;
  const int order_entry = ((ConstIntPtr)(unsigned long long)a.grp_order)[blockIdx.x];
  double R[9], t[3];
#pragma unroll
  for (int i = 0; i < 9; ++i) R[i] = st->hot.xi.R[i];
#pragma unroll
  for (int i = 0; i < 3; ++i) t[i] = st->hot.xi.t[i];
  float Tf[12];
#pragma unroll
  for (int i = 0; i < 12; ++i) Tf[i] = st->xi_f[i];
  asm volatile("" ::"s"(done_now), "s"(have_lin_now), "s"(cur), "s"(lin_unneeded_now), "s"(order_is_valid), "s"(order_entry), "s"(Tf[0]), "s"(Tf[11]), "s"(R[0]), "s"(t[2]));
  if (!(a.mode & 4) && done_now) return;

  const bool do_err = (a.mode & 1) && have_lin_now;
  const bool do_lin = (a.mode & 2);
  const float4* __restrict__ tpt_old = a.tpt[cur];
  const double* __restrict__ mahal_old = a.mahal[cur];
  float4* __restrict__ tpt_new = a.tpt[nxt];
  double* __restrict__ mahal_new = a.mahal[nxt];
  const Grid& g = a.grid;

  double wave_total = 0.0;
  unsigned int ncand = 0, nvalid = 0, nstaged = 0;

  const int lane = threadIdx.x & 63, wave = __builtin_amdgcn_readfirstlane((int)(threadIdx.x >> 6));
  const int sub = lane % G, grp = lane / G;
  WaveStage& S = stage_all[wave];
  NG_STAMP(0);
  const int group = order_is_valid ? order_entry : (int)blockIdx.x;
  const unsigned long long t_start = a.grp_cost ? __builtin_amdgcn_s_memtime() : 0ull;
  if (a.dbg_span && threadIdx.x == 0) a.dbg_span[(size_t)blockIdx.x * 4] = __builtin_amdgcn_s_memrealtime();
  if (a.t_first && blockIdx.x == 0 && threadIdx.x == 0 && !have_lin_now) *a.t_first = __builtin_amdgcn_s_memrealtime();
  if ((a.mode & 64) && lin_unneeded_now) {
    const int item = group * 4 + wave;
    double term = 0.0;
    if (item < a.n_batches) {
      typedef const int __attribute__((address_space(4))) * ConstBatchPtr;
      ConstBatchPtr brec = (ConstBatchPtr)(unsigned long long)a.batches + 2 * (size_t)item;
      const int qbase = brec[0], qcount = brec[1];
      if (lane < qcount) {
        const int i = qbase + lane;
        const float4 sp = a.qpts[i];
        float4 bp_old = make_float4(0.f, 0.f, 0.f, 0.f);
        int j_old = -1;
        double Mold[6] = {0, 0, 0, 0, 0, 0};
        if (have_lin_now) {
          bp_old = tpt_old[i];
          j_old = __float_as_int(bp_old.w);
        }
        if (do_err) {
          const double* M = mahal_old + (size_t)i * 6;
#pragma unroll
          for (int e = 0; e < 6; ++e) Mold[e] = M[e];
        }
        double k4 = 0.0;
        if (do_err && j_old >= 0) {
          const double ax = (double)sp.x, ay = (double)sp.y, az = (double)sp.z;
          const double tax = R[0] * ax + R[1] * ay + R[2] * az + t[0];
          const double tay = R[3] * ax + R[4] * ay + R[5] * az + t[1];
          const double taz = R[6] * ax + R[7] * ay + R[8] * az + t[2];
          const double ex = (double)bp_old.x - tax, ey = (double)bp_old.y - tay, ez = (double)bp_old.z - taz;
          if constexpr (ROBUST) k4 = err_term_robust(a.robust_kind, a.robust_c, a.robust_c2, ex, ey, ez, Mold);
          else k4 = err_term(ex, ey, ez, Mold);
        }
        term += k4;
      }
    }
    double* red = S.red;
    if (lane < 32) red[lane] = term;
    wave_lds_sync();
    if (lane < kNumSlots) {
      double out = 0.0;
      if (lane == 28)
        for (int l = 0; l < 32; ++l) out += red[l];
      wave_total += out;
      lds[wave][lane] = lane == 28 ? wave_total : 0.0;
    }
    __syncthreads();
    if (threadIdx.x < kNumSlots) {
      const int v = threadIdx.x;
      const double val = ((lds[0][v] + lds[1][v]) + lds[2][v]) + lds[3][v];
      if (FUSED) __hip_atomic_store(a.partials + (size_t)group * kNumSlots + v, val, __ATOMIC_RELAXED, __HIP_MEMORY_SCOPE_AGENT);
      else a.partials[(size_t)group * kNumSlots + v] = val;
    }
    if (a.dbg_span && threadIdx.x == 0) {
      unsigned long long* d = a.dbg_span + (size_t)blockIdx.x * 4;
      d[1] = __builtin_amdgcn_s_memrealtime();
      d[3] = (unsigned long long)(unsigned int)group;
    }
    if constexpr (!FUSED) return;
  } else {
#define NG_HAVE_LIN have_lin_now
#define NG_ROBUST ROBUST
#include "ngicp_pass_group.inc"
#undef NG_ROBUST
#undef NG_HAVE_LIN
  }
  if constexpr (FUSED) {
  if (wave == 0) {
    asm volatile("s_waitcnt vmcnt(0)" ::: "memory");
    if (lane == 0) {
      const int tk = __hip_atomic_fetch_add(a.ticket, 1, __ATOMIC_RELAXED, __HIP_MEMORY_SCOPE_AGENT);
      last_block = (tk == (int)gridDim.x - 1) ? 1 : 0;
    }
  }
  __syncthreads();
  if (!last_block) return;
  if (threadIdx.x == 0) {
    __hip_atomic_store(a.ticket, 0, __ATOMIC_RELAXED, __HIP_MEMORY_SCOPE_AGENT);
    __builtin_amdgcn_fence(__ATOMIC_ACQUIRE, "agent");
    asm volatile("s_waitcnt vmcnt(0)" ::: "memory");
  }
  __syncthreads();
  lm_solve_body<256, true>(a.sa, shm.sv);
  }
}

#include "ngicp_pass_routes.h"
#undef NG_STAMP

}
#include "ngicp_pass_st.h"
namespace ngk {

__global__ void __launch_bounds__(256) k_corr_to_original(const float4* __restrict__ tpt, const float4* __restrict__ qpts, const float4* __restrict__ src_sorted,
                                                           const float4* __restrict__ tgt_sorted, int n, int* __restrict__ out_corr, float* __restrict__ out_sqd,
                                                           const float* __restrict__ lin_f) {
  const int i = blockIdx.x * blockDim.x + threadIdx.x;
  if (i >= n) return;
  const float4 sp = qpts[i];
  const int o = __float_as_int(src_sorted[__float_as_int(sp.w)].w);
  const int j = __float_as_int(tpt[i].w);
  out_corr[o] = j >= 0 ? __float_as_int(tgt_sorted[j].w) : -1;
  if (out_sqd) {
    float d = __builtin_inff();
    if (j >= 0) {
      const float3 q = transform_point_rowmajor_f(lin_f, sp.x, sp.y, sp.z);
      d = sqdist(q.x, q.y, q.z, tgt_sorted[j]);
    }
    out_sqd[o] = d;
  }
}

}
```

direct_lidar_odometry_amd/csrc/ngicp_pass_group.inc:

```
#ifndef NG_ROBUST
#define NG_ROBUST false
#define NG_ROBUST_DEFAULTED
#endif
  for (int item = group * 4 + wave; item < a.n_batches; item = a.n_batches) {
    typedef const int __attribute__((address_space(4))) * ConstBatchPtr;
    ConstBatchPtr brec = (ConstBatchPtr)(unsigned long long)a.batches + 2 * (size_t)item;
    const int2 it = make_int2(brec[0], brec[1]);
    typedef const float __attribute__((address_space(4))) * ConstBoxPtr;
    const unsigned int far_word = (unsigned int)((ConstBatchPtr)(unsigned long long)a.batch_far)[item >> 2];
    const bool far_before = ((far_word >> (8 * (item & 3))) & 0xffu) != 0;
    ConstBoxPtr bbp = (ConstBoxPtr)(unsigned long long)a.batch_boxes + 6 * (size_t)item;
    const float bb_c0 = bbp[0], bb_c1 = bbp[1], bb_c2 = bbp[2], bb_h0 = bbp[3], bb_h1 = bbp[4], bb_h2 = bbp[5];
    const int qbase = it.x, qcount = it.y, batch = item;
    float mybest = 3.4028234664e38f;
    int mypos = -1;
    const int i = qbase + lane;
    const bool mine = lane < qcount;
    NG_STAMP(1);
    const bool have_prev = NG_HAVE_LIN != 0;
    float4 sp = make_float4(0.f, 0.f, 0.f, 0.f);
    int j_old = -1;
    float4 bp_old = make_float4(0.f, 0.f, 0.f, 0.f);
    double k4 = 0.0;
    double Mold[6] = {0, 0, 0, 0, 0, 0};
    if (mine) {
      sp = a.qpts[i];
      if (have_prev) {
        bp_old = tpt_old[i];
        j_old = __float_as_int(bp_old.w);
      }
      if (do_err) {
        const double* M = mahal_old + (size_t)i * 6;
#pragma unroll
        for (int e = 0; e < 6; ++e) Mold[e] = M[e];
      }
    }
    int Y0 = 0, Z0 = 0, wy = 1, grow = 0, nlive = 0;
    int b0x = 0, b0y = 0, b0z = 0, b1x = 0, b1y = 0, b1z = 0;
    bool list_rows = false;
    int rs[kStageRowsPerLane], rn[kStageRowsPerLane], rho[kStageRowsPerLane], ryz[kStageRowsPerLane], rk[kStageRowsPerLane];
    if (do_lin && !(a.mode & 8) && a.stage_grow >= 2 && (have_prev ? far_before : (a.mode & 32) != 0)) {
      {
        const float bcx = bb_c0, bcy = bb_c1, bcz = bb_c2, bhx = bb_h0, bhy = bb_h1, bhz = bb_h2;
        const float3 m = transform_point_rowmajor_f(Tf, bcx, bcy, bcz);
        const float mx = m.x, my = m.y, mz = m.z;
        const float pad = 1e-3f * g.h;
        const float ex = (fabsf(Tf[0]) * bhx + fabsf(Tf[1]) * bhy) + fabsf(Tf[2]) * bhz + pad + 4e-6f * (fabsf(mx) + bhx + bhy + bhz);
        const float ey = (fabsf(Tf[4]) * bhx + fabsf(Tf[5]) * bhy) + fabsf(Tf[6]) * bhz + pad + 4e-6f * (fabsf(my) + bhx + bhy + bhz);
        const float ez = (fabsf(Tf[8]) * bhx + fabsf(Tf[9]) * bhy) + fabsf(Tf[10]) * bhz + pad + 4e-6f * (fabsf(mz) + bhx + bhy + bhz);
        cell_coords(g, mx - ex, my - ey, mz - ez, b0x, b0y, b0z);
        cell_coords(g, mx + ex, my + ey, mz + ez, b1x, b1y, b1z);
      }
      int rows, X0 = 0, XS = 1;
      for (grow = a.stage_grow;; --grow) {
        X0 = max(b0x - grow, 0);
        Y0 = max(b0y - grow, 0);
        Z0 = max(b0z - grow, 0);
        const int X1 = min(b1x + grow, g.nx - 1), Y1 = min(b1y + grow, g.ny - 1), Z1 = min(b1z + grow, g.nz - 1);
        XS = X1 - X0 + 1;
        wy = Y1 - Y0 + 1;
        rows = wy * (Z1 - Z0 + 1);
        if ((rows <= kStageRows && XS <= kStageXs) || grow == 2) break;
      }
      if (rows <= kStageRows && XS <= kStageXs) {
        int sv[kStageRowsPerLane], ev[kStageRowsPerLane], ka[kStageRowsPerLane], kb[kStageRowsPerLane];
#pragma unroll
        for (int k = 0; k < kStageRowsPerLane; ++k) {
          const int r = lane + 64 * k;
          const bool has = r < rows;
          const int ry = Y0 + (has ? r : 0) % wy, rz = Z0 + (has ? r : 0) / wy;
          const int* rowp = a.tgt_cell_start + ((rz * g.ny + ry) * g.nx + X0);
          sv[k] = rowp[0];
          ev[k] = rowp[XS];
          ka[k] = rowp[b0x - X0];
          kb[k] = rowp[b1x + 1 - X0];
          rho[k] = max(max(b0y - ry, ry - b1y), max(max(b0z - rz, rz - b1z), 0));
          ryz[k] = ry | (rz << 16);
        }
        static_assert(kStageRowsPerLane == 4, "the four rows of a lane, spelled out for the compiler");
        asm volatile("" ::"v"(sv[0]), "v"(sv[1]), "v"(sv[2]), "v"(sv[3]), "v"(kb[0]), "v"(kb[1]), "v"(kb[2]), "v"(kb[3]));
#pragma unroll
        for (int k = 0; k < kStageRowsPerLane; ++k) {
          const bool has = lane + 64 * k < rows;
          rs[k] = sv[k];
          rn[k] = has ? ev[k] - sv[k] : 0;
          rk[k] = min(ka[k] - sv[k], 0xffff) | (min(kb[k] - sv[k], 0xffff) << 16);
        }
        list_rows = true;
      }
    }
    if (mine) {
      if (do_err && j_old >= 0) {
        const double ax = (double)sp.x, ay = (double)sp.y, az = (double)sp.z;
        const double tax = R[0] * ax + R[1] * ay + R[2] * az + t[0];
        const double tay = R[3] * ax + R[4] * ay + R[5] * az + t[1];
        const double taz = R[6] * ax + R[7] * ay + R[8] * az + t[2];
        const double ex = (double)bp_old.x - tax, ey = (double)bp_old.y - tay, ez = (double)bp_old.z - taz;
        if constexpr (NG_ROBUST) {
          k4 = err_term_robust(a.robust_kind, a.robust_c, a.robust_c2, ex, ey, ez, Mold);
        } else {
        const double m00 = Mold[0], m01 = Mold[1], m02 = Mold[2], m11 = Mold[3], m12 = Mold[4], m22 = Mold[5];
        const double mex = m00 * ex + m01 * ey + m02 * ez;
        const double mey = m01 * ex + m11 * ey + m12 * ez;
        const double mez = m02 * ex + m12 * ey + m22 * ez;
        k4 = ex * mex + ey * mey + ez * mez;
        }
      }
    }

    if (do_lin && (a.mode & 8)) {
      mypos = (qbase + lane) % 1000;
      mybest = 0.01f;
    } else if (do_lin) {
      const int qi = qbase + grp;
      const bool qok = grp < qcount;
      const float qpx = __shfl(sp.x, grp), qpy = __shfl(sp.y, grp), qpz = __shfl(sp.z, grp);
      const int jp = __shfl(j_old, grp);
      float4 bpo;
      bpo.x = __shfl(bp_old.x, grp); bpo.y = __shfl(bp_old.y, grp); bpo.z = __shfl(bp_old.z, grp); bpo.w = 0.f;
      float qx = 0.f, qy = 0.f, qz = 0.f;
      int cx = 0, cy = 0, cz = 0;
      if (qok) {
        const float3 q = transform_point_rowmajor_f(Tf, qpx, qpy, qpz);
        qx = q.x, qy = q.y, qz = q.z;
        cell_coords(g, qx, qy, qz, cx, cy, cz);
      }
      float best = 3.4028234664e38f;
      int pos = -1;
      if (qok && jp >= 0) {
        best = sqdist(qx, qy, qz, bpo);
        pos = jp;
      }
      NG_STAMP(2);
      bool listed = false;
      if (list_rows) {
        {
          wave_lds_sync();
          for (int lev = 0; lev <= grow; ++lev) {
#pragma unroll
            for (int k = 0; k < kStageRowsPerLane; ++k) {
              const bool on = rn[k] > 0 && rho[k] == lev;
              const unsigned long long m = __ballot(on);
              if (on) S.live[nlive + __popcll(m & ((1ull << lane) - 1ull))] = make_int4(ryz[k], rn[k], rs[k], rk[k]);
              nlive += __popcll(m);
            }
          }
          listed = true;
        }
      }
      NG_STAMP(3);
      if (a.dbg_stamps && lane == 0) {
        unsigned long long* d = a.dbg_stamps + (size_t)(blockIdx.x * 4 + wave) * kStampStride;
        d[10] = (unsigned long long)(listed ? grow : 0);
        d[11] = (unsigned long long)nlive;
        d[12] = (unsigned long long)qcount;
// ... 102 lines not shown
          if (tail <= kWalkers) return tail;
          if constexpr (kWalkLanes == 1) {
            return atomicAdd(&S.q_head, 1);
          } else {
            int nu = 0;
            if (ql == 0) nu = atomicAdd(&S.q_head, 1);
            return quad_perm_i<0x00>(nu);
          }
        };
        for (int u = lane / kWalkLanes; u < tail; u = next_unit()) {
          ++popped;
          const int uq = S.unit_q[u], qs = uq & 31, s0 = S.unit_s[u], e0 = S.unit_e[u];
          const float gyz = S.unit_g[u];
          const float4 q = S.qtab[qs];
          const unsigned long long k0 = S.qkey[qs];
          float ub = __uint_as_float((unsigned int)(k0 >> 32));
          int up = (int)(unsigned int)k0;
          if (gyz > fminf(ub, a.gate_sq_f)) continue;
          const unsigned int c_before = ncand;
          const unsigned int steps_before1 = dbg_g1;
          if constexpr (kWalkLanes == 1) scan_global_outward<kWin, kSideStep>(a.tgt3, s0, e0, s0 + (uq >> 9), q.x, q.y, q.z, gyz, a.gate_sq_f, ub, up, ncand, dbg_g1);
          else scan_quad_outward<kWin, kSideStep>(a.tgt3, s0, e0, s0 + (uq >> 9), q.x, q.y, q.z, gyz, a.gate_sq_f, ub, up, ncand, dbg_g1, ql);
          if (ql == 0) {
            if (a.dbg_qstats) atomicAdd(reinterpret_cast<int*>(a.dbg_qstats + a.n_src) + min((int)((dbg_g1 - steps_before1) & 0xffff), 63), 1);
            atomicMin(&S.qkey[qs], pack_key(ub, up));
            if (a.dbg_qstats) {
              atomicAdd(&S.qstat[qs][0], (int)(ncand - c_before));
              atomicAdd(&S.qstat[qs][1], 1);
            }
          }
        }
        NG_STAMP(17);
        if (a.dbg_stamps) {
          unsigned long long* d = a.dbg_stamps + (size_t)(blockIdx.x * 4 + wave) * kStampStride;
          atomicMax(&d[18], (unsigned long long)popped);
          if (lane == 0) d[19] = (unsigned long long)tail;
        }
      }
      wave_lds_sync();
      if (qok) {
        const unsigned long long k1 = S.qkey[grp];
        best = __uint_as_float((unsigned int)(k1 >> 32));
        pos = (int)(unsigned int)k1;
      }
      NG_STAMP(4);
      float bound1 = 0.f;
      if (qok) {
        bound1 = unexplored_bound_sq(g, qx, qy, qz, cx, cy, cz, 1);
        went_far = !(best <= bound1 || bound1 >= a.gate_sq_f);
      }
      const unsigned int dbg_c1 = ncand;
      unsigned int dbg_rows = 0;
      const bool need_far = in_box && went_far;
      if (listed && __any(need_far && (!pre_far || li_pre < nlive))) {
        int li = pre_far ? li_pre : sub;
        bool more = need_far;
        for (;;) {
          if (lane == 0) S.q_tail = 0, S.q_head = 0;
          wave_lds_sync();
          if (more) {
            const float lim = fminf(best, a.gate_sq_f);
            for (; li < nlive; li += G) {
              const int4 rec = S.live[li];
              if (row_gap_sq(g, rec.x & 0xffff, rec.x >> 16, cy, cz, qy, qz) > lim) continue;
              const int slot = atomicAdd(&S.q_tail, 1);
              if (slot >= kUnitCap) break;
              S.unit_q[slot] = grp | (li << 5);
              ++dbg_rows;
            }
            more = li < nlive;
          }
          wave_lds_sync();
          {
            const int tail = min(S.q_tail, kUnitCap);
            const int ql = lane % kWalkLanes;
            for (;;) {
              int u = 0;
              if (ql == 0) u = atomicAdd(&S.q_head, 1);
              if constexpr (kWalkLanes > 1) u = quad_perm_i<0x00>(u);
              if (u >= tail) break;
              const int unit = S.unit_q[u], qs = unit & 31;
              const int4 rec = S.live[unit >> 5];
              const float4 q = S.qtab[qs];
              int ux, uy, uz;
              cell_coords(g, q.x, q.y, q.z, ux, uy, uz);
              const float gyz = row_gap_sq(g, rec.x & 0xffff, rec.x >> 16, uy, uz, q.y, q.z);
              const unsigned long long k0 = S.qkey[qs];
              float ub = __uint_as_float((unsigned int)(k0 >> 32));
              int up = (int)(unsigned int)k0;
              if (gyz > fminf(ub, a.gate_sq_f)) continue;
              const int s0 = rec.z + (rec.w & 0xffff), e0 = rec.z + (int)((unsigned int)rec.w >> 16);
              const float frac3 = fminf(fmaxf((q.x - (g.ox + (float)b0x * g.h)) / ((float)(b1x + 1 - b0x) * g.h), 0.f), 1.f);
              const unsigned int c_before = ncand;
              const unsigned int steps_before2 = dbg_g2;
              if constexpr (kWalkLanes == 1) scan_global_outward<kWin, kSideStep>(a.tgt3, rec.z, rec.z + rec.y, s0 + (int)(frac3 * (float)(e0 - s0)), q.x, q.y, q.z, gyz, a.gate_sq_f, ub, up, ncand, dbg_g2);
              else scan_quad_outward<kWin, kSideStep>(a.tgt3, rec.z, rec.z + rec.y, s0 + (int)(frac3 * (float)(e0 - s0)), q.x, q.y, q.z, gyz, a.gate_sq_f, ub, up, ncand, dbg_g2, ql);
              if (ql == 0) {
                if (a.dbg_qstats) atomicAdd(reinterpret_cast<int*>(a.dbg_qstats + a.n_src) + 64 + min((int)((dbg_g2 - steps_before2) & 0xffff), 63), 1);
                atomicMin(&S.qkey[qs], pack_key(ub, up));
                if (a.dbg_qstats) {
                  atomicAdd(&S.qstat[qs][2], (int)(ncand - c_before));
                  atomicAdd(&S.qstat[qs][1], 1 << 16);
                }
              }
            }
          }
          wave_lds_sync();
          if (in_box) {
            const unsigned long long k1 = S.qkey[grp];
            best = __uint_as_float((unsigned int)(k1 >> 32));
            pos = (int)(unsigned int)k1;
          }
          if (!__any(more)) break;
        }
      }
      NG_STAMP(5);
      if (a.dbg_stamps && qok) {
        unsigned long long* d = a.dbg_stamps + (size_t)(blockIdx.x * 4 + wave) * kStampStride;
        atomicMax(&d[14], ((unsigned long long)(dbg_g2 & 0xffff) << 48) | ((unsigned long long)(dbg_g2 >> 16) << 32) | ((unsigned long long)dbg_rows << 16) | (ncand - dbg_c1));
        atomicMax(&d[15], ((unsigned long long)(dbg_g1 & 0xffff) << 48) | ((unsigned long long)(dbg_g1 >> 16) << 32) | dbg_c1);
      }
      const unsigned int c_before_shells = ncand;
      if (qok) nn_shells<G>(g, a.tgt3, a.tgt_cell_start, qx, qy, qz, cx, cy, cz, a.gate_sq_f, sub, need_far ? grow : 1, best, pos, ncand);
      if (a.dbg_qstats) {
        if (qok) atomicAdd(&S.qstat[grp][2], (int)(ncand - c_before_shells));
        wave_lds_sync();
        if (qok && sub == 0) a.dbg_qstats[qi] = make_int4(S.qstat[grp][0], S.qstat[grp][1], S.qstat[grp][2], (went_far ? 1 : 0) | (in_box ? 2 : 0) | (pos >= 0 ? 4 : 0));
      }
      {
        const bool any_far = __any(went_far);
        if (lane == 0) a.batch_far[batch] = any_far ? 1 : 0;
      }
      NG_STAMP(6);
      const int src_lane = (lane % B) * G;
      mybest = __shfl(best, src_lane);
      mypos = __shfl(pos, src_lane);
    }
    double acc[kNumSums];
#pragma unroll
    for (int v = 0; v < kNumSums; ++v) acc[v] = 0.0;
    if ((a.mode & 16) && mine) {
      tpt_new[i] = make_float4(0.f, 0.f, 0.f, __int_as_float(mypos));
      acc[27] += (double)mybest;
    } else if (mine) {
      const double ax = (double)sp.x, ay = (double)sp.y, az = (double)sp.z;
      const double tax = R[0] * ax + R[1] * ay + R[2] * az + t[0];
      const double tay = R[3] * ax + R[4] * ay + R[5] * az + t[1];
      const double taz = R[6] * ax + R[7] * ay + R[8] * az + t[2];

      acc[28] += k4;
      if (do_lin) {
        const int pos = mypos;
        const bool valid = (pos >= 0) && ((double)mybest < a.gate_sq);
        if (!valid) tpt_new[i] = make_float4(0.f, 0.f, 0.f, __int_as_float(-1));
        if (valid) {
          ++nvalid;
          const double* CB = a.cov_tgt + (size_t)pos * 6;
          const double* CA = a.cov_src + (size_t)__float_as_int(sp.w) * 6;
          const Xyz bp = a.tgt3[pos];
          double ca[6];
#pragma unroll
          for (int e = 0; e < 6; ++e) ca[e] = CA[e];
          tpt_new[i] = make_float4(bp.x, bp.y, bp.z, __int_as_float(pos));
          double rcr[6], M[6];
          rotate_sym(R, ca, rcr);
#pragma unroll
          for (int e = 0; e < 6; ++e) rcr[e] = CB[e] + rcr[e];
          inv3_sym(rcr, M);
          double* Mo = mahal_new + (size_t)i * 6;
#pragma unroll
          for (int e = 0; e < 6; ++e) Mo[e] = M[e];

          const double ex = (double)bp.x - tax, ey = (double)bp.y - tay, ez = (double)bp.z - taz;
          if constexpr (NG_ROBUST) lin_terms_robust(acc, a.robust_kind, a.robust_c, a.robust_c2, tax, tay, taz, ex, ey, ez, M);
          else lin_terms(acc, tax, tay, taz, ex, ey, ez, M);
        }
      }
    }
    {
      double* red = S.red;
      double out = 0.0;
#pragma unroll
      for (int half = 0; half < 2; ++half) {
        wave_lds_sync();
        if ((lane >> 4) == half) {
#pragma unroll
          for (int v = 0; v < kNumSums; ++v) red[(lane & 15) * 30 + v] = acc[v];
        }
        wave_lds_sync();
        if (lane < kNumSums)
          for (int l = 0; l < 16; ++l) out += red[l * 30 + lane];
      }
      if (lane < kNumSums) wave_total += out;
    }
  }

  NG_STAMP(7);
  {
    wave_lds_sync();
    unsigned int* cnt = reinterpret_cast<unsigned int*>(S.red);
    cnt[lane] = ncand;
    cnt[64 + lane] = nvalid;
    cnt[128 + lane] = nstaged;
    wave_lds_sync();
    if (lane >= kNumSums && lane < kNumSlots) {
      unsigned int sum = 0;
      for (int l = 0; l < 64; ++l) sum += cnt[(lane - kNumSums) * 64 + l];
      wave_total = (double)sum;
    }
    if (lane < kNumSlots) lds[wave][lane] = wave_total;
  }
  NG_STAMP(8);
  __syncthreads();
  NG_STAMP(9);
  if (threadIdx.x < kNumSlots) {
    const int v = threadIdx.x;
    const double val = ((lds[0][v] + lds[1][v]) + lds[2][v]) + lds[3][v];
    if (FUSED) __hip_atomic_store(a.partials + (size_t)group * kNumSlots + v, val, __ATOMIC_RELAXED, __HIP_MEMORY_SCOPE_AGENT);
    else a.partials[(size_t)group * kNumSlots + v] = val;
  }
  if (a.dbg_span && threadIdx.x == 0) {
    unsigned long long* d = a.dbg_span + (size_t)blockIdx.x * 4;
    d[1] = __builtin_amdgcn_s_memrealtime();
    d[2] = (unsigned long long)__builtin_amdgcn_s_getreg((31 << 11) | 4) | ((unsigned long long)__builtin_amdgcn_s_getreg((31 << 11) | 20) << 32);
    d[3] = (unsigned long long)(unsigned int)group;
  }
  if (a.grp_cost && threadIdx.x == 0) {
    const int cost = (int)min((__builtin_amdgcn_s_memtime() - t_start) >> 4, 0x7fffffffull);
    if (FUSED) __hip_atomic_store(a.grp_cost + group, cost, __ATOMIC_RELAXED, __HIP_MEMORY_SCOPE_AGENT);
    else a.grp_cost[group] = cost;
  }
#ifdef NG_ROBUST_DEFAULTED
#undef NG_ROBUST
#undef NG_ROBUST_DEFAULTED
#endif
```

direct_lidar_odometry_amd/csrc/ngicp_search.h:

```cpp
#pragma once
#include "ngicp_grid.h"

namespace ngk {

struct alignas(4) Xyz { float x, y, z; };
__device__ __forceinline__ float sqdist(float qx, float qy, float qz, const Xyz& p) {
  const float dx = qx - p.x, dy = qy - p.y, dz = qz - p.z;
  float r = dx * dx;
  r = r + dy * dy;
  r = r + dz * dz;
  return r;
}

__device__ __forceinline__ float3 transform_point_rowmajor_f(const float* Tf, float x, float y, float z) {
  float3 q;
  q.x = ((Tf[0] * x + Tf[1] * y) + Tf[2] * z) + Tf[3];
  q.y = ((Tf[4] * x + Tf[5] * y) + Tf[6] * z) + Tf[7];
  q.z = ((Tf[8] * x + Tf[9] * y) + Tf[10] * z) + Tf[11];
  return q;
}

__global__ void __launch_bounds__(256) k_pack_pos(const float4* __restrict__ in, int n_padded, int pad, float4* __restrict__ out) {
  const int i = blockIdx.x * blockDim.x + threadIdx.x;
  if (i >= n_padded) return;
  const float4 p = in[i];
  const bool real = i >= pad && i < n_padded - pad;
  out[i] = make_float4(p.x, p.y, p.z, __int_as_float(real ? i - pad : -1));
}

__global__ void __launch_bounds__(256) k_pack_xyz(const float4* __restrict__ in, int n, Xyz* __restrict__ out) {
  const int i = blockIdx.x * blockDim.x + threadIdx.x;
  if (i >= n) return;
  const float4 p = in[i];
  out[i] = Xyz{p.x, p.y, p.z};
}

template <int G>
__device__ __forceinline__ void group_min(float& d, int& p) {
#pragma unroll
  for (int o = G / 2; o > 0; o >>= 1) {
    const float od = __shfl_xor(d, o);
    const int op = __shfl_xor(p, o);
    const bool take = (od < d) || (od == d && (unsigned)op < (unsigned)p);
    d = take ? od : d;
    p = take ? op : p;
  }
}

__device__ __forceinline__ bool nn_better(float d, int p, float best, int bestp) { return d < best || (d == best && (unsigned)p < (unsigned)bestp); }

constexpr int kStageRowsPerLane = 4;
constexpr int kStageRows = 64 * kStageRowsPerLane;
constexpr int kStageXs = 20;
constexpr int kStageMaxGrow = 6;

#ifndef NGICP_PASS_WAVES
#define NGICP_PASS_WAVES 3
#endif
#ifndef NGICP_WALK_WINDOW
#define NGICP_WALK_WINDOW 12
#endif

#ifndef NGICP_WALK_PREFETCH
#define NGICP_WALK_PREFETCH 0
#endif
#ifndef NGICP_PRE_FAR
#define NGICP_PRE_FAR 0
#endif
#ifndef NGICP_ALIGNED_WINDOWS
#define NGICP_ALIGNED_WINDOWS 0
#endif
constexpr int kWalkWindow = NGICP_WALK_WINDOW;
static_assert(kWalkWindow <= kSortedPad && kWalkWindow % 2 == 0, "walk windows may overhang the array by at most the sentinel frame");

constexpr int kUnitCap = 288;

struct WaveStage {
  union {
    struct {
      int4 live[kStageRows];
      int qstat[32][3];
    };
    double red[16 * 30];
  };
  unsigned long long qkey[32];
  float4 qtab[32];
  int unit_q[kUnitCap], unit_s[kUnitCap], unit_e[kUnitCap];
  float unit_g[kUnitCap];
  int q_tail, q_head;
};

__device__ __forceinline__ void wave_lds_sync() {
  __builtin_amdgcn_fence(__ATOMIC_RELEASE, "wavefront");
  __builtin_amdgcn_wave_barrier();
  __builtin_amdgcn_fence(__ATOMIC_ACQUIRE, "wavefront");
}

template <int W = kWalkWindow, int kStep = kWalkWindow, class PT>
__device__ __forceinline__ void scan_global_outward(const PT* __restrict__ tgt, int s, int e, int m, float qx, float qy, float qz, float gyz, float gate_sq,
                                                    float& best, int& pos, unsigned int& ncand, unsigned int& gsteps) {
  if (e <= s) return;
  gsteps += 0x10000u;
  m = min(max(m, s), e - 1);
  constexpr bool kQuadLoads = NGICP_ALIGNED_WINDOWS && sizeof(PT) == 12 && W % 4 == 0 && kStep % 4 == 0;
  const int w0 = kQuadLoads ? ((m - W / 2) & ~3) : m - W / 2;
  int w = w0, dir = 0, lo = w0, hi = w0 + W;
  int wn = W;
  static_assert(kStep >= 2 && kStep <= W, "side windows are at most as long as the first");
  bool go_left = false;
  for (;;) {
    const PT* __restrict__ q = tgt + w;
    PT c[W];
    if constexpr (kQuadLoads) {
      const float4* __restrict__ q4 = reinterpret_cast<const float4*>(q);
      float4 r[3 * W / 4];
#pragma unroll
      for (int j = 0; j < 3 * W / 4; ++j)
        if (j < 3 * kStep / 4 || wn == W) r[j] = q4[j];
#pragma unroll
      for (int j = 0; j < W / 4; ++j) {
        if (j < kStep / 4 || wn == W) {
          const float4 r0 = r[3 * j], r1 = r[3 * j + 1], r2 = r[3 * j + 2];
          c[4 * j].x = r0.x; c[4 * j].y = r0.y; c[4 * j].z = r0.z;
          c[4 * j + 1].x = r0.w; c[4 * j + 1].y = r1.x; c[4 * j + 1].z = r1.y;
          c[4 * j + 2].x = r1.z; c[4 * j + 2].y = r1.w; c[4 * j + 2].z = r2.x;
          c[4 * j + 3].x = r2.y; c[4 * j + 3].y = r2.z; c[4 * j + 3].z = r2.w;
        }
      }
    } else {
#pragma unroll
      for (int j = 0; j < W; ++j)
        if (j < kStep || wn == W) c[j] = q[j];
    }
    unsigned int pf = 0;
    if constexpr (NGICP_WALK_PREFETCH != 0) {
      if (dir >= 0 && hi < e) pf ^= *reinterpret_cast<const unsigned int*>(tgt + (hi + (NGICP_WALK_PREFETCH > 1 ? kStep - 1 : 0)));
      if (dir <= 0 && lo > s) pf ^= *reinterpret_cast<const unsigned int*>(tgt + (lo - (NGICP_WALK_PREFETCH > 1 ? kStep : 1)));
    }
    float lb = sqdist(qx, qy, qz, c[0]);
    int lj = 0;
#pragma unroll
    for (int j = 1; j < W; ++j) {
      if (j < kStep || wn == W) {
        const float d = sqdist(qx, qy, qz, c[j]);
        if (d < lb) { lb = d; lj = j; }
      }
    }
    if (nn_better(lb, w + lj, best, pos)) { best = lb; pos = w + lj; }
    ncand += wn;
    ++gsteps;
    if constexpr (NGICP_WALK_PREFETCH != 0) gsteps += (pf == 0x7fc0beefu) ? 0x100u : 0u;
    const float lim = fminf(best, gate_sq), dr = (wn == W ? c[W - 1].x : c[kStep - 1].x) - qx, dl = qx - c[0].x;
    const bool more_right = hi < e && !(dr > 0.f && dr * dr + gyz > lim);
    const bool more_left = lo > s && !(dl > 0.f && dl * dl + gyz > lim);
    if (dir == 0) go_left = more_left;
    if (dir >= 0 && more_right) {
      dir = 1;
      w = hi;
      hi += kStep;
      wn = kStep;
    } else if (dir >= 0 ? go_left : more_left) {
      dir = -1;
      lo -= kStep;
      w = lo;
      wn = kStep;
    } else {
      break;
    }
  }
}

#ifndef NGICP_WALK_LANES
#define NGICP_WALK_LANES 1
#endif
constexpr int kWalkLanes = NGICP_WALK_LANES;
template <int CTRL>
__device__ __forceinline__ int quad_perm_i(int v) { return __builtin_amdgcn_update_dpp(v, v, CTRL, 0xf, 0xf, false); }
template <int CTRL>
__device__ __forceinline__ float quad_perm_f(float v) { return __int_as_float(quad_perm_i<CTRL>(__float_as_int(v))); }
template <int W, int kStep, class PT>
__device__ __forceinline__ void scan_quad_outward(const PT* __restrict__ tgt, int s, int e, int m, float qx, float qy, float qz, float gyz, float gate_sq,
                                                  float& best, int& pos, unsigned int& ncand, unsigned int& gsteps, int ql) {
  static_assert(W % 4 == 0 && kStep % 4 == 0 && kStep >= 4 && kStep <= W, "windows are dealt to the four lanes of a quad");
  constexpr int PER = W / 4, PERS = kStep / 4;
  if (e <= s) return;
  gsteps += 0x10000u;
  m = min(max(m, s), e - 1);
  int w = m - W / 2, dir = 0, lo = m - W / 2, hi = m - W / 2 + W;
  int wn = W;
  bool go_left = false;
  for (;;) {
    const PT* __restrict__ q = tgt + (w + ql);
    PT c[PER];
#pragma unroll
    for (int j = 0; j < PER; ++j)
      if (j < PERS || wn == W) c[j] = q[4 * j];
    float lb = sqdist(qx, qy, qz, c[0]);
    int lj = 0;
#pragma unroll
    for (int j = 1; j < PER; ++j) {
      if (j < PERS || wn == W) {
        const float d = sqdist(qx, qy, qz, c[j]);
        if (d < lb) { lb = d; lj = j; }
      }
    }
    int lp = w + ql + 4 * lj;
    const float xl = quad_perm_f<0x00>(c[0].x), xr = quad_perm_f<0xff>(wn == W ? c[PER - 1].x : c[PERS - 1].x);
    {
      const float od = quad_perm_f<0xb1>(lb);
      const int op = quad_perm_i<0xb1>(lp);
      if (nn_better(od, op, lb, lp)) { lb = od; lp = op; }
    }
    {
      const float od = quad_perm_f<0x4e>(lb);
      const int op = quad_perm_i<0x4e>(lp);
      if (nn_better(od, op, lb, lp)) { lb = od; lp = op; }
    }
    if (nn_better(lb, lp, best, pos)) { best = lb; pos = lp; }
    if (ql == 0) ncand += wn;
    ++gsteps;
    const float lim = fminf(best, gate_sq), dr = xr - qx, dl = qx - xl;
    const bool more_right = hi < e && !(dr > 0.f && dr * dr + gyz > lim);
    const bool more_left = lo > s && !(dl > 0.f && dl * dl + gyz > lim);
    if (dir == 0) go_left = more_left;
// ... 70 lines not shown
```

direct_lidar_odometry_amd/csrc/ngicp_solve.h:

```cpp
#pragma once
#include "ngicp_lm.h"

namespace ngk {

constexpr int kSolveSubs = kSolveThreads / 16;
#ifndef NGICP_SOLVE_CHUNK
#define NGICP_SOLVE_CHUNK 40
#endif
constexpr int kSolveChunk = NGICP_SOLVE_CHUNK;


template <int THREADS>
struct SolveShared {
  double wsum[32][kPartialStride];
  double sums[kPartialStride];
  int ord_cnt[THREADS / 64 - 1][16], ord_pos[THREADS / 64 - 1][16];
  int ord_cost[kMaxOrderGroups];
  unsigned char ord_cls[kMaxOrderGroups];
  int ord_arrived;
  LmHot L;
};

template <int THREADS>
__device__ __forceinline__ void build_launch_order(const SolveArgs& a, SolveShared<THREADS>& sh, const int lane, const int wave) {
  auto& ord_cnt = sh.ord_cnt;
  auto& ord_pos = sh.ord_pos;
  auto& ord_cost = sh.ord_cost;
  auto& ord_cls = sh.ord_cls;
  int& ord_arrived = sh.ord_arrived;
  const unsigned long long t_ord = a.dbg_stamps ? __builtin_amdgcn_s_memtime() : 0ull;
  constexpr int kSortWaves = THREADS / 64 - 1;
  const int sw = wave - 1;
  auto wsync = [] {
    __builtin_amdgcn_fence(__ATOMIC_RELEASE, "wavefront");
    __builtin_amdgcn_wave_barrier();
    __builtin_amdgcn_fence(__ATOMIC_ACQUIRE, "wavefront");
  };
  auto same_class = [&](int cls, bool valid) -> unsigned long long {
    unsigned long long m = __ballot(valid);
#pragma unroll
    for (int bit = 0; bit < 4; ++bit) {
      const bool one = (cls >> bit) & 1;
      const unsigned long long bb = __ballot(valid && one);
      m &= one ? bb : ~bb;
    }
    return m;
  };
  if (lane < 16) ord_cnt[sw][lane] = 0;
  int mx = 1;
  for (int gi = lane; gi < a.nblocks; gi += 64) mx = max(mx, ord_cost[gi]);
#pragma unroll
  for (int o = 32; o > 0; o >>= 1) mx = max(mx, __shfl_xor(mx, o));
  const float to_class = 16.0f / ((float)mx + 1.0f);
  const unsigned long long lt = (1ull << lane) - 1ull;
  const int slice = ((a.nblocks + kSortWaves * 64 - 1) / (kSortWaves * 64)) * 64;
  const int g_first = sw * slice, g_last = min(g_first + slice, a.nblocks);
  wsync();
  for (int g0 = g_first; g0 < g_last; g0 += 64) {
    const int gi = g0 + lane;
    const bool valid = gi < g_last;
    const int cls = valid ? 15 - min(15, (int)((float)ord_cost[gi] * to_class)) : 0;
    if (valid) ord_cls[gi] = (unsigned char)cls;
    const unsigned long long m = same_class(cls, valid);
    if (valid && (m & lt) == 0) ord_cnt[sw][cls] += __popcll(m);
    wsync();
  }
  __builtin_amdgcn_fence(__ATOMIC_RELEASE, "workgroup");
  if (lane == 0) atomicAdd(&ord_arrived, 1);
  bool met = false;
  for (int spin = 0; spin < (1 << 20); ++spin) {
    if (*reinterpret_cast<volatile int*>(&ord_arrived) >= kSortWaves) {
      met = true;
      break;
    }
    __builtin_amdgcn_s_sleep(2);
  }
  __builtin_amdgcn_fence(__ATOMIC_ACQUIRE, "workgroup");
  if (met) {
    if (lane < 16) {
      int run = 0;
      for (int c = 0; c < lane; ++c)
        for (int w = 0; w < kSortWaves; ++w) run += ord_cnt[w][c];
      for (int w = 0; w < sw; ++w) run += ord_cnt[w][lane];
      ord_pos[sw][lane] = run;
    }
    wsync();
    for (int g0 = g_first; g0 < g_last; g0 += 64) {
      const int gi = g0 + lane;
      const bool valid = gi < g_last;
      const int cls = valid ? ord_cls[gi] : 0;
      const unsigned long long m = same_class(cls, valid);
      const int base = ord_pos[sw][cls];
      if (valid) a.grp_order[base + __popcll(m & lt)] = gi;
      wsync();
      if (valid && (m & lt) == 0) ord_pos[sw][cls] = base + __popcll(m);
      wsync();
    }
    if (sw == 0 && lane == 0 && a.order_valid) *a.order_valid = 1;
  }
  if (a.dbg_stamps && sw == 0 && lane == 0) a.dbg_stamps[7] = __builtin_amdgcn_s_memtime() - t_ord;
}

template <int THREADS, bool AGENT, bool PERSIST = false>
__device__ __forceinline__ void lm_solve_body(const SolveArgs& a, SolveShared<THREADS>& sh) {
  static_assert(!PERSIST || AGENT, "the persistent solver is an agent-scope one");
  constexpr int kSolveThreads = THREADS;
  constexpr int kSolveSubs = 32;
  constexpr int kThreadSubs = THREADS / 16;
  constexpr int kPer = kSolveSubs / kThreadSubs;
  constexpr int kSolveChunk = THREADS >= 512 ? NGICP_SOLVE_CHUNK : 14;
  static_assert(kPer >= 1 && kPer * kThreadSubs == kSolveSubs, "block sizes: 256 or 512 threads");
  auto& wsum = sh.wsum;
  auto& sums = sh.sums;
  auto& ord_cost = sh.ord_cost;
  int& ord_arrived = sh.ord_arrived;
  LmHot& L = sh.L;
  if (threadIdx.x == 0) ord_arrived = 0;
  LmState* st = a.st;
  LmState* sto = a.st_out ? a.st_out : a.st;
#define NG_SSTAMP(k)                                                                 \
  do {                                                                               \
    if (a.dbg_stamps && threadIdx.x == 0) a.dbg_stamps[k] = __builtin_amdgcn_s_memtime(); \
  } while (0)
  const int done_at_entry = PERSIST ? 0 : __hip_atomic_load(&st->hot.done, __ATOMIC_RELAXED, __HIP_MEMORY_SCOPE_WORKGROUP);
  const unsigned long long t_solver_entry = a.dbg_stamps ? __builtin_amdgcn_s_memtime() : 0ull;
  const int lane = threadIdx.x & 63, wave = threadIdx.x >> 6;
  const int vp = threadIdx.x & 15, sb = threadIdx.x >> 4;
  const double2* __restrict__ rows = reinterpret_cast<const double2*>(a.partials) + vp;
  static_assert(sizeof(LmHot) % 4 == 0, "LmHot is copied as dwords");
  constexpr int kHotWords = (int)(sizeof(LmHot) / 4), kHotPerThread = (kHotWords + kSolveThreads - 1) / kSolveThreads;
  constexpr int kCostPerThread = kMaxOrderGroups / kSolveThreads;
  const int passes_at_entry = PERSIST ? __hip_atomic_load(&st->hot.passes, __ATOMIC_RELAXED, __HIP_MEMORY_SCOPE_AGENT) : st->hot.passes;
  const int k4_only_at_entry = (!PERSIST && a.pass_honours_word) ? st->hot.lin_unneeded : 0;
  const bool order_it = a.mode == 0 && a.grp_order && a.nblocks <= kMaxOrderGroups && !k4_only_at_entry && (PERSIST ? passes_at_entry == 2 : (!AGENT || passes_at_entry < 3 || (passes_at_entry & 3) == 3));
  int hv[kHotPerThread];
#pragma unroll
  for (int k = 0; k < kHotPerThread; ++k) {
    const int w = threadIdx.x + k * kSolveThreads;
    if constexpr (PERSIST) hv[k] = w < kHotWords ? __hip_atomic_load(reinterpret_cast<const int*>(&st->hot) + w, __ATOMIC_RELAXED, __HIP_MEMORY_SCOPE_AGENT) : 0;
    else hv[k] = w < kHotWords ? reinterpret_cast<const int*>(&st->hot)[w] : 0;
  }
  const int last_row = (a.nrows ? a.nrows : a.nblocks) - 1, last_grp = a.nblocks - 1;
  auto load_row = [](const double2* q) -> double2 {
    if constexpr (PERSIST) {
      const double* d = reinterpret_cast<const double*>(q);
      return make_double2(__hip_atomic_load(d, __ATOMIC_RELAXED, __HIP_MEMORY_SCOPE_AGENT), __hip_atomic_load(d + 1, __ATOMIC_RELAXED, __HIP_MEMORY_SCOPE_AGENT));
    } else {
      return *q;
    }
  };
  double2 p[kPer * kSolveChunk];
#pragma unroll
  for (int sI = 0; sI < kPer; ++sI)
#pragma unroll
    for (int j = 0; j < kSolveChunk; ++j) {
      const int gi = sb + sI * kThreadSubs + j * kSolveSubs;
      p[sI * kSolveChunk + j] = gi <= last_row ? load_row(rows + (size_t)gi * (kNumSlots / 2)) : make_double2(0.0, 0.0);
    }
  int oc[kCostPerThread];
#pragma unroll
  for (int k = 0; k < kCostPerThread; ++k) {
    const int gi = threadIdx.x + k * kSolveThreads;
    if constexpr (PERSIST) oc[k] = (order_it && gi <= last_grp) ? __hip_atomic_load(a.grp_cost + gi, __ATOMIC_RELAXED, __HIP_MEMORY_SCOPE_AGENT) : 0;
    else oc[k] = (order_it && gi <= last_grp) ? a.grp_cost[gi] : 0;
  }
  double prior_v = 0.0;
  if (a.prior && threadIdx.x < kPriorDoubles) prior_v = a.prior[threadIdx.x];
  if (a.mode == 0 && done_at_entry) return;
  if (a.dbg_stamps && threadIdx.x == 0) a.dbg_stamps[0] = t_solver_entry;
#pragma unroll
  for (int k = 0; k < kHotPerThread; ++k) {
    const int w = threadIdx.x + k * kSolveThreads;
    if (w < kHotWords) reinterpret_cast<int*>(&L)[w] = hv[k];
  }
  if (order_it) {
#pragma unroll
    for (int k = 0; k < kCostPerThread; ++k) {
      const int gi = threadIdx.x + k * kSolveThreads;
      if (gi < a.nblocks) ord_cost[gi] = oc[k];
    }
  }
  {
    double a0[kPer], a1[kPer];
#pragma unroll
    for (int sI = 0; sI < kPer; ++sI) {
      a0[sI] = p[sI * kSolveChunk].x;
      a1[sI] = p[sI * kSolveChunk].y;
#pragma unroll
      for (int j = 1; j < kSolveChunk; ++j) {
        a0[sI] += p[sI * kSolveChunk + j].x;
        a1[sI] += p[sI * kSolveChunk + j].y;
      }
    }
    for (int g0 = kSolveSubs * kSolveChunk; g0 + sb <= last_row; g0 += kSolveSubs * kSolveChunk) {
#pragma unroll
      for (int sI = 0; sI < kPer; ++sI)
#pragma unroll
        for (int j = 0; j < kSolveChunk; ++j) {
          const int gi = g0 + sb + sI * kThreadSubs + j * kSolveSubs;
          p[sI * kSolveChunk + j] = gi <= last_row ? load_row(rows + (size_t)gi * (kNumSlots / 2)) : make_double2(0.0, 0.0);
        }
#pragma unroll
      for (int sI = 0; sI < kPer; ++sI)
#pragma unroll
        for (int j = 0; j < kSolveChunk; ++j) {
          a0[sI] += p[sI * kSolveChunk + j].x;
          a1[sI] += p[sI * kSolveChunk + j].y;
        }
    }
    NG_SSTAMP(1);
#pragma unroll
    for (int sI = 0; sI < kPer; ++sI) {
      wsum[sb + sI * kThreadSubs][2 * vp] = a0[sI];
      wsum[sb + sI * kThreadSubs][2 * vp + 1] = a1[sI];
    }
  }
  __syncthreads();
  if (threadIdx.x < kPartialStride) {
    const int v = threadIdx.x;
    double t = 0.0;
    if (v < kNumSlots)
      for (int sb = 0; sb < kSolveSubs; ++sb) t += wsum[sb][v];
    sums[v] = t;
  }
  __syncthreads();
  NG_SSTAMP(2);
  if (a.sums_out && threadIdx.x < kPartialStride) a.sums_out[threadIdx.x] = sums[threadIdx.x];
  if (a.mode == 3) return;
  if (order_it && wave >= 1) build_launch_order<THREADS>(a, sh, lane, wave);
  if (wave != 0) return;
  if (a.prior) {
    double* const P = &wsum[0][0];
    if (lane < kPriorDoubles) P[lane] = prior_v;
    wave_sync();
    double r[6], theta_sq, jc;
    prior_residual(L.xi, P, r, theta_sq, jc);
    if (lane < 36) P[kPriorDoubles + lane] = prior_jac_elem(lane / 6, lane % 6, r[0], r[1], r[2], theta_sq, jc, L.xi.t[0], L.xi.t[1], L.xi.t[2]);
#pragma unroll
    for (int q = 0; q < 6; ++q)
      if (lane == 36 + q) P[kPriorDoubles + 36 + q] = r[q];
    wave_sync();
    if (lane < kPriorRowSums + 1) sums[lane] += prior_row_elem(lane < kPriorRowSums ? lane : kPriorRowSums - 1, P + kPriorDoubles, P + 12, P + kPriorDoubles + 36);
    wave_sync();
  }
  if (a.mode == 2) {
    if (lane == 0) st->hot.y0 = sums[28];
    return;
  }
  if (a.mode != 1 && !a.serial_step) {
    NG_SSTAMP(3);
    lm_step_wave(L, a.cfg, sums, a.trace, a.max_trace_rows, !(a.pass_honours_word && L.lin_unneeded), lane);
    NG_SSTAMP(4);
    wave_sync();
    NG_SSTAMP(5);
    if (!L.done && lane < 12) {
      const float f = (float)reinterpret_cast<const double*>(&L.xi)[lane];
      if constexpr (PERSIST) __hip_atomic_store(&st->xi_f[pose_elem_to_rows(lane)], f, __ATOMIC_RELAXED, __HIP_MEMORY_SCOPE_AGENT);
      else sto->xi_f[pose_elem_to_rows(lane)] = f;
    }
  } else if (lane == 0) {
    if (a.mode == 1) {
      adopt_new(L, sums);
    } else {
      const LmConfig& cfg = a.cfg;
      NG_SSTAMP(3);
      lm_step(L, cfg, sums, a.trace, a.max_trace_rows, !(a.pass_honours_word && L.lin_unneeded));
      NG_SSTAMP(4);
      NG_SSTAMP(5);
      if (!L.done) {
#pragma unroll
        for (int r = 0; r < 3; ++r) {
#pragma unroll
          for (int c = 0; c < 4; ++c) {
            const float f = (float)(c < 3 ? L.xi.R[r * 3 + c] : L.xi.t[r]);
            if constexpr (PERSIST) __hip_atomic_store(&st->xi_f[r * 4 + c], f, __ATOMIC_RELAXED, __HIP_MEMORY_SCOPE_AGENT);
            else sto->xi_f[r * 4 + c] = f;
          }
        }
      }
    }
  }
  if (a.mode == 0 && lane == 0 && L.done) {
    L.t_done = __builtin_amdgcn_s_memrealtime();
    if (a.t_first) L.t_first = PERSIST ? __hip_atomic_load(a.t_first, __ATOMIC_RELAXED, __HIP_MEMORY_SCOPE_AGENT) : *a.t_first;
  }
  __builtin_amdgcn_fence(__ATOMIC_RELEASE, "wavefront");
  __builtin_amdgcn_wave_barrier();
  __builtin_amdgcn_fence(__ATOMIC_ACQUIRE, "wavefront");
  const bool finished_now = a.mode == 0 && L.done != 0;
  if constexpr (!PERSIST) {
    for (int w = lane; w < (int)(sizeof(LmHot) / 4); w += 64) reinterpret_cast<int*>(&sto->hot)[w] = reinterpret_cast<const int*>(&L)[w];
  }
  if (finished_now && a.final_host) {
    for (int w = lane; w < (int)(sizeof(LmHot) / 4); w += 64)
      __hip_atomic_store(reinterpret_cast<int*>(a.final_host) + w, reinterpret_cast<const int*>(&L)[w], __ATOMIC_RELAXED, __HIP_MEMORY_SCOPE_SYSTEM);
    __threadfence_system();
    __builtin_amdgcn_wave_barrier();
  }
  if (a.mode == 0 && a.progress_host && lane == 0)
    __hip_atomic_store(a.progress_host, (L.passes & kProgressMask) | (L.done ? kProgressDone : 0), __ATOMIC_RELAXED, __HIP_MEMORY_SCOPE_SYSTEM);
  if constexpr (PERSIST) {
    for (int w = lane; w < (int)(sizeof(LmHot) / 4); w += 64)
      __hip_atomic_store(reinterpret_cast<int*>(&st->hot) + w, reinterpret_cast<const int*>(&L)[w], __ATOMIC_RELAXED, __HIP_MEMORY_SCOPE_AGENT);
    int v = 0;
    if (lane < 24) {
      v = reinterpret_cast<const int*>(&L.xi)[lane];
    } else if (lane < 36) {
      const int r = (lane - 24) >> 2, cI = (lane - 24) & 3;
      v = __float_as_int((float)(cI < 3 ? L.xi.R[r * 3 + cI] : L.xi.t[r]));
    } else if (lane == kViewDone) {
      v = L.done;
    } else if (lane == kViewCur) {
      v = L.cur;
    } else if (lane == kViewHaveLin) {
      v = L.have_lin;
    }
    __hip_atomic_store(st->view + (size_t)L.passes * kViewWords + lane, v, __ATOMIC_RELAXED, __HIP_MEMORY_SCOPE_AGENT);
  }
  NG_SSTAMP(6);
#undef NG_SSTAMP
}

__global__ void __launch_bounds__(kSolveThreads) k_lm_solve(SolveArgs a) {
  __shared__ SolveShared<kSolveThreads> sh;
  lm_solve_body<kSolveThreads, false>(a, sh);
}

constexpr int kStepSelftestIn = 132;
constexpr size_t kStepSelftestRecord = sizeof(LmHot) + 18 * sizeof(double);
static_assert(sizeof(LmHot) % 8 == 0, "the trace row behind the image is 8-byte aligned");
__global__ void __launch_bounds__(64) k_step_selftest(const double* __restrict__ in, int n_problems, unsigned char* __restrict__ out) {
  __shared__ LmHot L;
  __shared__ double sums[kPartialStride];
  static_assert(kPartialStride >= 32, "32 reduced sums");
  const int lane = threadIdx.x;
  if ((int)blockIdx.x >= n_problems) return;
  const double* p = in + (size_t)blockIdx.x * kStepSelftestIn;
  LmConfig cfg;
  cfg.max_iterations = (int)p[93];
  cfg.lm_max_iterations = (int)p[94];
  cfg.optimizer = (int)p[95];
  cfg.rot_eps = p[96];
  cfg.trans_eps = p[97];
  cfg.lm_init_lambda_factor = p[98];
  const bool searched = p[131] != 0.0;
  for (int form = 0; form < 2; ++form) {
    unsigned char* rec = out + ((size_t)blockIdx.x * 2 + form) * kStepSelftestRecord;
    double* tail = reinterpret_cast<double*>(rec + sizeof(LmHot));
    __syncthreads();
    for (int w = lane; w < (int)(sizeof(LmHot) / 4); w += 64) reinterpret_cast<int*>(&L)[w] = 0;
    if (lane < 32) sums[lane] = p[99 + lane];
    __syncthreads();
    if (lane < 36) reinterpret_cast<double*>(&L.x0)[lane] = p[lane];
    if (lane < 36) L.H[lane] = p[36 + lane];
    if (lane < 6) L.b[lane] = p[72 + lane], L.d[lane] = p[79 + lane];
    if (lane == 0) {
      L.y0 = p[78];
      L.lambda = p[85];
      L.nu = p[86];
      L.iter = (int)p[87];
      L.trial = (int)p[88];
      L.have_lin = (int)p[89];
      L.cur = (int)p[90];
      L.n_trace = max(0, (int)p[91]);
      L.lin_unneeded = (int)p[92];
    }
    __syncthreads();
    if (form == 0) {
      if (lane == 0) lm_step(L, cfg, sums, tail, 1, searched);
    } else {
      lm_step_wave(L, cfg, sums, tail, 1, searched, lane);
    }
    __syncthreads();
    for (int w = lane; w < (int)(sizeof(LmHot) / 4); w += 64) reinterpret_cast<int*>(rec)[w] = reinterpret_cast<const int*>(&L)[w];
    if (lane < 6) tail[8 + lane] = L.d[lane];
    if (lane == 0) tail[14] = L.done, tail[15] = L.converged, tail[16] = L.lm_failed, tail[17] = L.trial;
  }
}
static_assert(offsetof(LmHot, xi) == offsetof(LmHot, x0) + sizeof(Pose) && offsetof(LmHot, delta) == offsetof(LmHot, xi) + sizeof(Pose), "x0, xi, delta are contiguous");

}
```

direct_lidar_odometry_amd/csrc/ngicp_voxel.h:

```cpp
#pragma once
#include "ngicp_pass.h"

namespace ngk {

constexpr int kVoxBias = 1 << 20;
constexpr int kVoxKeyBits = 63;
constexpr unsigned long long kVoxEmpty = ~0ull;
constexpr int kVoxBlock = 256;
constexpr int kVoxRec = 10;

__device__ __forceinline__ bool voxel_cell(float x, float y, float z, float inv_res, int& ix, int& iy, int& iz) {
  const float fx = floorf(x * inv_res), fy = floorf(y * inv_res), fz = floorf(z * inv_res);
  const float lim = 1048576.f;
  if (!(fx > -lim && fx < lim && fy > -lim && fy < lim && fz > -lim && fz < lim)) return false;
  ix = (int)fx, iy = (int)fy, iz = (int)fz;
  return true;
}

__device__ __forceinline__ unsigned long long voxel_pack(int ix, int iy, int iz) {
  return ((unsigned long long)(iz + kVoxBias) << 42) | ((unsigned long long)(iy + kVoxBias) << 21) | (unsigned long long)(ix + kVoxBias);
}

__device__ __forceinline__ bool voxel_key(float x, float y, float z, float inv_res, unsigned long long& key) {
  int ix, iy, iz;
// ... 134 lines not shown
                                                           unsigned long long* __restrict__ vkeys, ulonglong2* __restrict__ table, unsigned int mask) {
  const int v = blockIdx.x * blockDim.x + threadIdx.x;
  if (v >= n_vox) return;
  const int s = seg_start[v], e = seg_start[v + 1];
  double S[kVoxRec];
  for (int j = s; j < e; ++j) {
    const int g = order[j];
    int lo = 0, hi = m;
    while (hi - lo > 1) {
      const int mid = (lo + hi) >> 1;
      if (part_off[mid] <= g) lo = mid;
      else hi = mid;
    }
    const double* r = part_rec[lo] + (size_t)(g - part_off[lo]) * kVoxRec;
    if (j == s) {
#pragma unroll
      for (int k = 0; k < kVoxRec; ++k) S[k] = r[k];
    } else {
#pragma unroll
      for (int k = 0; k < kVoxRec; ++k) S[k] = S[k] + r[k];
    }
  }
  voxel_record_from_sums(S, rec + (size_t)v * kVoxRec);
  const unsigned long long key = keys[s];
  vkeys[v] = key;
  voxel_table_insert(table, mask, key, v);
}

struct VoxelPassArgs {
  const float4* src;
  const double* cov_src;
  int n_src;
  const ulonglong2* table;
  unsigned int mask;
  const double* rec;
  int n_vox;
  float inv_res;
  int* corr[2];
  double* mahal[2];
  LmState* st;
  double* partials;
  int mode;
  unsigned long long* t_first;
  int nbr;
  int slot_stride;
  int robust_kind;
  double robust_c, robust_c2;
};

struct VoxelPassLds {
  double red[4][16 * 30];
  double lds[4][kNumSlots];
  unsigned int cnt[4][2][64];
};

__device__ __forceinline__ void voxel_block_row(const double (&acc)[kNumSums], const unsigned int nprobes, const unsigned int nvalid, VoxelPassLds& sh, double* partials) {
  double (&lds)[4][kNumSlots] = sh.lds;
  unsigned int (&cnt)[4][2][64] = sh.cnt;
  const int lane = threadIdx.x & 63, wave = threadIdx.x >> 6;
  {
    double* rw = sh.red[wave];
    double out = 0.0;
#pragma unroll
    for (int q = 0; q < 4; ++q) {
      wave_lds_sync();
      if ((lane >> 4) == q) {
#pragma unroll
        for (int v = 0; v < kNumSums; ++v) rw[(lane & 15) * 30 + v] = acc[v];
      }
      wave_lds_sync();
      if (lane < kNumSums)
        for (int l = 0; l < 16; ++l) out += rw[l * 30 + lane];
    }
    cnt[wave][0][lane] = nprobes;
    cnt[wave][1][lane] = nvalid;
    wave_lds_sync();
    if (lane >= kNumSums && lane < kNumSums + 2) {
      unsigned int sum = 0;
      for (int l = 0; l < 64; ++l) sum += cnt[wave][lane - kNumSums][l];
      out = (double)sum;
    }
    if (lane < kNumSlots) lds[wave][lane] = lane < kNumSums + 2 ? out : 0.0;
  }
  __syncthreads();
  if (threadIdx.x < kNumSlots) {
    const int v = threadIdx.x;
    partials[(size_t)blockIdx.x * kNumSlots + v] = ((lds[0][v] + lds[1][v]) + lds[2][v]) + lds[3][v];
  }
}

template <bool ROBUST = false, class A>
__device__ __forceinline__ void vgicp_pass_body(A& a, const PassPose& p, VoxelPassLds& sh) {
  const double (&R)[9] = p.R;
  const double (&t)[3] = p.t;
  const float (&Tf)[12] = p.Tf;
  const int cur = p.cur;
  const int nxt = cur ^ 1;
  const bool do_err = (a.mode & 1) && p.have_lin;
  const bool do_lin = (a.mode & 2);
  const int i = blockIdx.x * kVoxBlock + threadIdx.x;
  const bool mine = i < a.n_src;

  double acc[kNumSums];
#pragma unroll
  for (int v = 0; v < kNumSums; ++v) acc[v] = 0.0;
  unsigned int nprobes = 0, nvalid = 0;
  if (mine) {
    const float4 sp = a.src[i];
    const double ax = (double)sp.x, ay = (double)sp.y, az = (double)sp.z;
    const double tax = R[0] * ax + R[1] * ay + R[2] * az + t[0];
    const double tay = R[3] * ax + R[4] * ay + R[5] * az + t[1];
    const double taz = R[6] * ax + R[7] * ay + R[8] * az + t[2];
    if (do_err) {
      const int v_old = a.corr[cur][i];
      if ((unsigned int)v_old < (unsigned int)a.n_vox) {
        const double* mv = a.rec + (size_t)v_old * kVoxRec;
        if constexpr (ROBUST) acc[28] += err_term_robust(a.robust_kind, a.robust_c, a.robust_c2, mv[0] - tax, mv[1] - tay, mv[2] - taz, a.mahal[cur] + (size_t)i * 6);
        else acc[28] += err_term(mv[0] - tax, mv[1] - tay, mv[2] - taz, a.mahal[cur] + (size_t)i * 6);
      }
    }
    if (do_lin) {
      const float3 q = transform_point_rowmajor_f(Tf, sp.x, sp.y, sp.z);
      unsigned long long key = 0;
      int v = -1;
      if (voxel_key(q.x, q.y, q.z, a.inv_res, key)) v = voxel_lookup(a.table, a.mask, key, nprobes);
      a.corr[nxt][i] = v;
      if (v >= 0) {
        ++nvalid;
        const double* rv = a.rec + (size_t)v * kVoxRec;
        const double* CA = a.cov_src + (size_t)i * 6;
        double ca[6], rcr[6], M[6];
#pragma unroll
        for (int e = 0; e < 6; ++e) ca[e] = CA[e];
        const double bx = rv[0], by = rv[1], bz = rv[2], nv = rv[9];
        rotate_sym(R, ca, rcr);
#pragma unroll
        for (int e = 0; e < 6; ++e) rcr[e] = rv[3 + e] + rcr[e];
        inv3_sym(rcr, M);
#pragma unroll
        for (int e = 0; e < 6; ++e) M[e] = nv * M[e];
        double* Mo = a.mahal[nxt] + (size_t)i * 6;
#pragma unroll
        for (int e = 0; e < 6; ++e) Mo[e] = M[e];
        if constexpr (ROBUST) lin_terms_robust(acc, a.robust_kind, a.robust_c, a.robust_c2, tax, tay, taz, bx - tax, by - tay, bz - taz, M);
        else lin_terms(acc, tax, tay, taz, bx - tax, by - tay, bz - taz, M);
      }
    }
  }
  voxel_block_row(acc, nprobes, nvalid, sh, a.partials);
}

typedef const VoxelPassArgs __attribute__((address_space(4))) KernelVoxelPassArgs;

__device__ __forceinline__ bool voxel_pass_begin(const VoxelPassArgs& a, PassPose& p) {
  const LmState* __restrict__ st = a.st;
  const int done_now = st->hot.done;
  load_pose(st, p);
  if (!(a.mode & 4) && done_now) return false;
  if (a.t_first && blockIdx.x == 0 && threadIdx.x == 0 && !p.have_lin) *a.t_first = __builtin_amdgcn_s_memrealtime();
  return true;
}

template <bool ROBUST = false>
__global__ void __launch_bounds__(kVoxBlock) k_vgicp_pass(VoxelPassArgs a) {
  __shared__ VoxelPassLds sh;
  PassPose p;
  if (!voxel_pass_begin(a, p)) return;
  vgicp_pass_body<ROBUST>(a, p, sh);
}

__global__ void __launch_bounds__(256) k_voxel_corr_to_original(const int* __restrict__ corr, const float4* __restrict__ src, int n, const double* __restrict__ rec,
                                                                 int* __restrict__ out_corr, float* __restrict__ out_sqd, const float* __restrict__ lin_f) {
  const int i = blockIdx.x * blockDim.x + threadIdx.x;
  if (i >= n) return;
  const float4 sp = src[i];
  const int o = __float_as_int(sp.w);
  const int v = corr[i];
  out_corr[o] = v;
  if (out_sqd) {
    float d = __builtin_inff();
    if (v >= 0) {
      const float3 q = transform_point_rowmajor_f(lin_f, sp.x, sp.y, sp.z);
      const double* mv = rec + (size_t)v * kVoxRec;
      d = sqdist(q.x, q.y, q.z, Xyz{(float)mv[0], (float)mv[1], (float)mv[2]});
    }
    out_sqd[o] = d;
  }
}

template <int K>
__host__ __device__ constexpr int vox_nbr_off(int s, int axis) {
  static_assert(K == 7 || K == 27, "DIRECT7 or DIRECT27");
  if (K == 27) return axis == 0 ? s % 3 - 1 : axis == 1 ? (s / 3) % 3 - 1 : s / 9 - 1;
  if (s == 0) return 0;
  return (s - 1) / 2 == axis ? (((s - 1) & 1) ? -1 : 1) : 0;
}
template <int K>
__host__ __device__ constexpr int vox_nbr_centre() { return K == 27 ? 13 : 0; }

template <int K>
struct VoxelPassLdsN : VoxelPassLds {
  int vs[K][kVoxBlock];
};

template <int K, bool ROBUST = false, class A>
__device__ __forceinline__ void vgicp_pass_n_body(A& a, const PassPose& p, VoxelPassLdsN<K>& sh) {
  const double (&R)[9] = p.R;
  const double (&t)[3] = p.t;
  const float (&Tf)[12] = p.Tf;
  const int cur = p.cur;
  int (&vs)[K][kVoxBlock] = sh.vs;
  const int nxt = cur ^ 1;
  const bool do_err = (a.mode & 1) && p.have_lin;
  const bool do_lin = (a.mode & 2);
  const int i = blockIdx.x * kVoxBlock + threadIdx.x;
  const bool mine = i < a.n_src;
  const size_t stride = (size_t)a.slot_stride;

  double acc[kNumSums];
#pragma unroll
  for (int v = 0; v < kNumSums; ++v) acc[v] = 0.0;
  unsigned int nprobes = 0, nvalid = 0;
  if (mine) {
    const float4 sp = a.src[i];
    const double ax = (double)sp.x, ay = (double)sp.y, az = (double)sp.z;
    const double tax = R[0] * ax + R[1] * ay + R[2] * az + t[0];
    const double tay = R[3] * ax + R[4] * ay + R[5] * az + t[1];
    const double taz = R[6] * ax + R[7] * ay + R[8] * az + t[2];
    if (do_err) {
      const int* __restrict__ co = a.corr[cur] + i;
      int vo[K];
#pragma unroll
      for (int s = 0; s < K; ++s) vo[s] = co[(size_t)s * stride];
#pragma unroll
      for (int s = 0; s < K; ++s) {
        if ((unsigned int)vo[s] < (unsigned int)a.n_vox) {
          const double* mv = a.rec + (size_t)vo[s] * kVoxRec;
          if constexpr (ROBUST) acc[28] += err_term_robust(a.robust_kind, a.robust_c, a.robust_c2, mv[0] - tax, mv[1] - tay, mv[2] - taz, a.mahal[cur] + ((size_t)s * stride + i) * 6);
          else acc[28] += err_term(mv[0] - tax, mv[1] - tay, mv[2] - taz, a.mahal[cur] + ((size_t)s * stride + i) * 6);
        }
      }
    }
    if (do_lin) {
      const float3 q = transform_point_rowmajor_f(Tf, sp.x, sp.y, sp.z);
      int cx, cy, cz;
      int* __restrict__ cn = a.corr[nxt] + i;
      if (!voxel_cell(q.x, q.y, q.z, a.inv_res, cx, cy, cz)) {
#pragma unroll
        for (int s = 0; s < K; ++s) cn[(size_t)s * stride] = -1;
      } else {
        unsigned long long key[K];
        ulonglong2 first[K];
        unsigned int in_range = 0;
#pragma unroll
        for (int s = 0; s < K; ++s) {
          const int nx = cx + vox_nbr_off<K>(s, 0), ny = cy + vox_nbr_off<K>(s, 1), nz = cz + vox_nbr_off<K>(s, 2);
          const bool ok = nx > -kVoxBias && nx < kVoxBias && ny > -kVoxBias && ny < kVoxBias && nz > -kVoxBias && nz < kVoxBias;
          key[s] = voxel_pack(nx, ny, nz);
          in_range |= ok ? (1u << s) : 0u;
          first[s] = a.table[ok ? voxel_hash(key[s], a.mask) : 0u];
        }
#pragma unroll
        for (int s = 0; s < K; ++s) {
          int v = -1;
          if (in_range & (1u << s)) {
            ++nprobes;
            if (first[s].x == key[s]) {
              v = (int)first[s].y;
            } else if (first[s].x != kVoxEmpty) {
              v = voxel_probe_from(a.table, a.mask, (voxel_hash(key[s], a.mask) + 1) & a.mask, key[s], nprobes);
            }
          }
          cn[(size_t)s * stride] = v;
          vs[s][threadIdx.x] = v;
        }
        const double* CA = a.cov_src + (size_t)i * 6;
        double ca[6], rcr[6];
#pragma unroll
        for (int e = 0; e < 6; ++e) ca[e] = CA[e];
        rotate_sym(R, ca, rcr);
#pragma unroll 1
        for (int s = 0; s < K; ++s) {
          const int v = vs[s][threadIdx.x];
          if (v < 0) continue;
          ++nvalid;
          const double* rv = a.rec + (size_t)v * kVoxRec;
          double S[6], M[6];
          const double bx = rv[0], by = rv[1], bz = rv[2], nv = rv[9];
#pragma unroll
          for (int e = 0; e < 6; ++e) S[e] = rv[3 + e] + rcr[e];
          inv3_sym(S, M);
#pragma unroll
          for (int e = 0; e < 6; ++e) M[e] = nv * M[e];
          double* Mo = a.mahal[nxt] + ((size_t)s * stride + i) * 6;
#pragma unroll
          for (int e = 0; e < 6; ++e) Mo[e] = M[e];
          if constexpr (ROBUST) lin_terms_robust(acc, a.robust_kind, a.robust_c, a.robust_c2, tax, tay, taz, bx - tax, by - tay, bz - taz, M);
          else lin_terms(acc, tax, tay, taz, bx - tax, by - tay, bz - taz, M);
        }
      }
    }
  }
  voxel_block_row(acc, nprobes, nvalid, sh, a.partials);
}

template <int K, bool ROBUST = false>
__global__ void __launch_bounds__(kVoxBlock, 2) k_vgicp_pass_n(VoxelPassArgs a) {
  __shared__ VoxelPassLdsN<K> sh;
  PassPose p;
  if (!voxel_pass_begin(a, p)) return;
  vgicp_pass_n_body<K, ROBUST>(a, p, sh);
}

__global__ void __launch_bounds__(256) k_voxel_corr_n_to_original(const int* __restrict__ corr, const float4* __restrict__ src, int n, int K, int slot_stride,
                                                                   int* __restrict__ out) {
  const int i = blockIdx.x * blockDim.x + threadIdx.x;
  if (i >= n) return;
  const int o = __float_as_int(src[i].w);
  for (int s = 0; s < K; ++s) out[(size_t)o * K + s] = corr[(size_t)s * slot_stride + i];
}

}
```

direct_lidar_odometry_amd/csrc/ngicp_voxel_batch.h:

```cpp
#pragma once
#include "ngicp_batch.h"
#include "ngicp_voxel.h"

namespace ngk {

template <int K>
struct VoxelBatchKernelTraits {
  typedef VoxelPassLdsN<K> Lds;
};
template <>
struct VoxelBatchKernelTraits<1> {
  typedef VoxelPassLds Lds;
};

template <int K>
__global__ void __launch_bounds__(kVoxBlock, K == 1 ? 1 : 2) k_vgicp_pass_batch(BatchLaunch bl) {
  static_assert(K == 1 || K == 7 || K == 27, "DIRECT1, DIRECT7 or DIRECT27");
  __shared__ typename VoxelBatchKernelTraits<K>::Lds sh;
  KernelBatchLaunch* kb = (KernelBatchLaunch*)__builtin_amdgcn_kernarg_segment_ptr();
  const int lane_id = kb->lane[blockIdx.y];
  KernelVoxelPassArgs* ka = (KernelVoxelPassArgs*)(unsigned long long)(reinterpret_cast<const VoxelPassArgs*>(kb->pass) + lane_id);
  KernelStatePtr st4 = (KernelStatePtr)(unsigned long long)ka->st;
  if (st4->hot.done) return;
  PassPose p;
  load_pose(st4, p);
  if constexpr (K == 1)
    vgicp_pass_body(*ka, p, sh);
  else
    vgicp_pass_n_body<K>(*ka, p, sh);
}

}
```

Baseline: 20850.

## Preload hot kernel pointers as leading kernargs and add optional write-through output stores

The pass, solve and batch kernels now take their most-used pointers (LM state, order flags, partials, per-lane record arrays) as separate leading kernel arguments, and the build enables kernarg preloading of the first eight dwords into SGPRs. The aim is to cut the scalar kernarg loads on each short launch's critical startup path. A compile-time switch also adds inline-asm global_store_dwordx4 with sc1 for the pass outputs. It is off in the default build, and a second library is built with it on. The extra padding arguments and inline asm add complexity and depend on the exact kernarg layout.

```diff
diff --git a/__graft_entry__.py b/__graft_entry__.py
--- a/__graft_entry__.py
+++ b/__graft_entry__.py
@@ -10,6 +10,7 @@
     from direct_lidar_odometry_amd import build as b
     lib = b.build()
     assert os.path.exists(lib)
+    assert os.path.exists(b.build_other_stores_variant())
     import direct_lidar_odometry_amd
     from direct_lidar_odometry_amd import nano_gicp
     L = nano_gicp.load_library()
diff --git a/direct_lidar_odometry_amd/build.py b/direct_lidar_odometry_amd/build.py
--- a/direct_lidar_odometry_amd/build.py
+++ b/direct_lidar_odometry_amd/build.py
@@ -11,7 +11,10 @@
 SOURCES = ["ngicp_api.hip", "ngicp_filters.hip"]
 PUBLIC_HEADER = os.path.normpath(os.path.join(HERE, "..", "include", "ngicp.h"))
 DEP_SUFFIXES = (".h", ".inc", ".hip")
-FLAGS = ["--offload-arch=gfx950", "-O3", "-std=c++17", "-ffp-contract=off", "-fPIC", "-shared", "-Wall", "-Wno-unused-function"]
+PASS_WT_STORES = 0
+OTHER_PASS_WT_STORES = 3 if PASS_WT_STORES == 0 else 0
+FLAGS = ["--offload-arch=gfx950", "-O3", "-std=c++17", "-ffp-contract=off", "-fPIC", "-shared", "-Wall", "-Wno-unused-function",
+         "-mllvm", "-amdgpu-kernarg-preload-count=8", f"-DNGICP_PASS_WT_STORES={PASS_WT_STORES}"]
 
 
 def hipcc() -> str:
@@ -26,18 +29,26 @@
     return sorted(found) + [PUBLIC_HEADER, os.path.abspath(__file__)]
 
 
-def needs_build() -> bool:
-    if not os.path.exists(LIB):
+def needs_build(lib: str = LIB) -> bool:
+    if not os.path.exists(lib):
         return True
-    t = os.path.getmtime(LIB)
+    t = os.path.getmtime(lib)
     return any(os.path.getmtime(d) > t for d in dependencies())
 
 
-def build(force: bool = False, verbose: bool = False, extra_flags: list[str] | None = None) -> str:
-    if not force and not needs_build():
-        return LIB
-    tmp = f"{LIB}.{os.getpid()}.tmp"
-    cmd = [hipcc(), *FLAGS, *(extra_flags or []), *[os.path.join(CSRC, s) for s in SOURCES], "-o", tmp]
+OTHER_STORES_LIB = os.path.join(HERE, "libngicp_hip.other_stores.so")
+
+
+def build_other_stores_variant(force: bool = False) -> str:
+    flags = [f"-DNGICP_PASS_WT_STORES={OTHER_PASS_WT_STORES}" if f.startswith("-DNGICP_PASS_WT_STORES=") else f for f in FLAGS]
+    return build(force=force, out=OTHER_STORES_LIB, flags=flags)
+
+
+def build(force: bool = False, verbose: bool = False, extra_flags: list[str] | None = None, out: str = LIB, flags: list[str] | None = None) -> str:
+    if not force and not needs_build(out):
+        return out
+    tmp = f"{out}.{os.getpid()}.tmp"
+    cmd = [hipcc(), *(flags or FLAGS), *(extra_flags or []), *[os.path.join(CSRC, s) for s in SOURCES], "-o", tmp]
     if verbose:
         print(" ".join(cmd), flush=True)
     res = subprocess.run(cmd, capture_output=True, text=True)
@@ -46,8 +57,8 @@
         raise RuntimeError("hipcc failed")
     if verbose and res.stderr:
         sys.stderr.write(res.stderr)
-    os.replace(tmp, LIB)
-    return LIB
+    os.replace(tmp, out)
+    return out
 
 
 if __name__ == "__main__":
diff --git a/direct_lidar_odometry_amd/csrc/ngicp_align.h b/direct_lidar_odometry_amd/csrc/ngicp_align.h
--- a/direct_lidar_odometry_amd/csrc/ngicp_align.h
+++ b/direct_lidar_odometry_amd/csrc/ngicp_align.h
@@ -40,7 +40,9 @@
 void launch_pass(ngicp* h, const PassArgs& a, const route::Variant& v, int nblocks, hipStream_t s, hipEvent_t start = nullptr, hipEvent_t stop = nullptr) {
   using K = void (*)(PassArgs);
   const bool four = v.waves == 4;
+  using KW = void (*)(const LmState*, const int*, const int*, KernargPad<40>, PassArgs);
   K kernel = nullptr;
+  KW walks = nullptr;
   PassArgs b = a;
   unsigned grid = (unsigned)nblocks;
   switch (v.family) {
@@ -56,12 +58,13 @@
       kernel = four ? K(k_gicp_queue<2, 4>) : K(k_gicp_queue<2, 3>);
       break;
     case route::Family::Walks:
-      if (v.fused) kernel = four ? K(k_gicp_pass<2, 4, true>) : K(k_gicp_pass<2, 3, true>);
-      else if (v.robust) kernel = four ? K(k_gicp_pass<2, 4, false, true>) : K(k_gicp_pass<2, 3, false, true>);
-      else kernel = four ? K(k_gicp_pass<2, 4>) : K(k_gicp_pass<2, 3>);
+      if (v.fused) walks = four ? KW(k_gicp_pass<2, 4, true>) : KW(k_gicp_pass<2, 3, true>);
+      else if (v.robust) walks = four ? KW(k_gicp_pass<2, 4, false, true>) : KW(k_gicp_pass<2, 3, false, true>);
+      else walks = four ? KW(k_gicp_pass<2, 4>) : KW(k_gicp_pass<2, 3>);
       break;
   }
-  hipExtLaunchKernelGGL(kernel, dim3(grid), dim3(256), 0, s, start, stop, 0, b);
+  if (walks) hipExtLaunchKernelGGL(walks, dim3(grid), dim3(256), 0, s, start, stop, 0, static_cast<const LmState*>(b.st), b.order_valid, b.grp_order, KernargPad<40>{}, b);
+  else hipExtLaunchKernelGGL(kernel, dim3(grid), dim3(256), 0, s, start, stop, 0, b);
 }
 
 struct LoopCtx {
@@ -613,7 +616,7 @@
         if (!route::row(pick.fallback).own_solver) return;
         SolveArgs sa = c.sa;
         if (stamp_launch > 1 && i + 1 != stamp_launch) sa.dbg_stamps = nullptr;
-        hipLaunchKernelGGL(k_lm_solve, dim3(1), dim3(kSolveThreads), 0, h->stream, sa);
+        launch_lm_solve(sa, h->stream);
       });
       break;
     }
@@ -651,8 +654,9 @@
   with_voxel_variant(c.pa.nbr, c.pa.robust_kind != NGICP_ROBUST_NONE, [&](auto k, auto robust) {
     constexpr int K = decltype(k)::value;
     constexpr bool R = decltype(robust)::value;
-    if constexpr (K == 1) hipExtLaunchKernelGGL(k_vgicp_pass<R>, grid, block, 0, h->stream, start, stop, 0, c.pa);
-    else hipExtLaunchKernelGGL((k_vgicp_pass_n<K, R>), grid, block, 0, h->stream, start, stop, 0, c.pa);
+    const LmState* st = c.pa.st;
+    if constexpr (K == 1) hipExtLaunchKernelGGL(k_vgicp_pass<R>, grid, block, 0, h->stream, start, stop, 0, st, c.pa);
+    else hipExtLaunchKernelGGL((k_vgicp_pass_n<K, R>), grid, block, 0, h->stream, start, stop, 0, st, c.pa);
   });
 }
 
@@ -712,7 +716,7 @@
   begin_alignment(h, al, guess, c.sa, c.pa.t_first);
   feed_alignment(h, al, max_passes(h->p), [&](long, hipEvent_t start, hipEvent_t stop) {
     launch_voxel_pass(h, c, start, stop);
-    hipLaunchKernelGGL(k_lm_solve, dim3(1), dim3(kSolveThreads), 0, h->stream, c.sa);
+    launch_lm_solve(c.sa, h->stream);
   });
   HIP_TRY(hipGetLastError());
   end_alignment(h, al, aligned, out_stride);
@@ -745,7 +749,7 @@
   }
   SolveArgs sa = k.vox ? k.vc.sa : k.c.sa;
   sa.mode = solve_mode;
-  hipLaunchKernelGGL(k_lm_solve, dim3(1), dim3(kSolveThreads), 0, h->stream, sa);
+  launch_lm_solve(sa, h->stream);
 }
 
 size_t round_up(size_t v, size_t a) { return (v + a - 1) / a * a; }
@@ -808,7 +812,7 @@
     idle_seen = false;
     for (int i = 0; i < n_live; ++i) bl.lane[i] = live[(size_t)i];
     launch_pass_batch(bl, n_live);
-    hipLaunchKernelGGL(k_lm_solve_batch, dim3((unsigned)n_live), dim3(kSolveThreads), 0, h->stream, bl);
+    hipLaunchKernelGGL(k_lm_solve_batch, dim3((unsigned)n_live), dim3(kSolveThreads), 0, h->stream, bl.solve, bl);
     ++launched;
   }
 }
@@ -936,9 +940,9 @@
   run_batch(h, r, T_out, converged, nr_iterations, hessians, [&](const BatchLaunch& l, int n_live) {
     const bool four = (long)nblocks * n_live > 2L * h->pass_slots;
     if (four)
-      hipLaunchKernelGGL((k_gicp_pass_batch<2, 4>), dim3((unsigned)nblocks, (unsigned)n_live), dim3(256), 0, h->stream, l);
+      hipLaunchKernelGGL((k_gicp_pass_batch<2, 4>), dim3((unsigned)nblocks, (unsigned)n_live), dim3(256), 0, h->stream, static_cast<const PassArgs*>(l.pass), l);
     else
-      hipLaunchKernelGGL((k_gicp_pass_batch<2, 3>), dim3((unsigned)nblocks, (unsigned)n_live), dim3(256), 0, h->stream, l);
+      hipLaunchKernelGGL((k_gicp_pass_batch<2, 3>), dim3((unsigned)nblocks, (unsigned)n_live), dim3(256), 0, h->stream, static_cast<const PassArgs*>(l.pass), l);
   });
   w.order_src = h->src.dev.get();
   w.order_groups = nblocks;
@@ -980,7 +984,7 @@
   }
   run_batch(h, r, T_out, converged, nr_iterations, hessians, [&](const BatchLaunch& l, int n_live) {
     const dim3 grid((unsigned)nblocks, (unsigned)n_live), block(kVoxBlock);
-    with_voxel_variant((int)K, false, [&](auto k, auto) { hipLaunchKernelGGL(k_vgicp_pass_batch<decltype(k)::value>, grid, block, 0, h->stream, l); });
+    with_voxel_variant((int)K, false, [&](auto k, auto) { hipLaunchKernelGGL(k_vgicp_pass_batch<decltype(k)::value>, grid, block, 0, h->stream, static_cast<const VoxelPassArgs*>(l.pass), l); });
   });
 }
 
diff --git a/direct_lidar_odometry_amd/csrc/ngicp_api.hip b/direct_lidar_odometry_amd/csrc/ngicp_api.hip
--- a/direct_lidar_odometry_amd/csrc/ngicp_api.hip
+++ b/direct_lidar_odometry_amd/csrc/ngicp_api.hip
@@ -1504,7 +1504,7 @@
     sa.mode = 3;
     sa.sums_out = sums32_dev;
     sa.grp_order = nullptr;
-    hipLaunchKernelGGL(k_lm_solve, dim3(1), dim3(kSolveThreads), 0, s, sa);
+    launch_lm_solve(sa, s);
     HIP_TRY(hipGetLastError());
   });
 }
@@ -1521,7 +1521,7 @@
     sa.partials = sums32_dev;
     sa.nblocks = 1;
     sa.grp_order = nullptr;
-    hipLaunchKernelGGL(k_lm_solve, dim3(1), dim3(kSolveThreads), 0, s, sa);
+    launch_lm_solve(sa, s);
     h->shard_stream = s;
     const long k = h->shard_steps++;
     const int slot = (int)(k % kShardSlots);
diff --git a/direct_lidar_odometry_amd/csrc/ngicp_batch.h b/direct_lidar_odometry_amd/csrc/ngicp_batch.h
--- a/direct_lidar_odometry_amd/csrc/ngicp_batch.h
+++ b/direct_lidar_odometry_amd/csrc/ngicp_batch.h
@@ -12,6 +12,14 @@
   int lane[kBatchMaxLanes];
 };
 typedef const BatchLaunch __attribute__((address_space(4))) KernelBatchLaunch;
+struct BatchKernargs {
+  const void* records;
+  BatchLaunch bl;
+};
+__device__ __forceinline__ KernelBatchLaunch* batch_launch_args() {
+  typedef const char __attribute__((address_space(4))) * ConstBytePtr;
+  return (KernelBatchLaunch*)((ConstBytePtr)__builtin_amdgcn_kernarg_segment_ptr() + offsetof(BatchKernargs, bl));
+}
 
 #define NG_STAMP(k) \
   do {              \
@@ -19,6 +27,7 @@
 template <int G, int WPS>
 __device__ __forceinline__ void batch_group_body(KernelPassArgs& a, const int group, WaveStage* stage_all, double (*lds)[kNumSlots]) {
   constexpr bool FUSED = false;
+  constexpr bool kWtOut = ((NGICP_PASS_WT_STORES >> (WPS >= 4 ? 1 : 0)) & 1) != 0;
   constexpr int B = 64 / G;
   constexpr int kWin = WPS >= 4 ? 12 : 16, kSideStep = WPS >= 4 ? 8 : 16;
   static_assert(kWin <= kSortedPad && B == kBatchQueries, "see k_gicp_pass");
@@ -56,18 +65,20 @@
   WaveStage& S = stage_all[wave];
   const unsigned long long t_start = a.grp_cost ? __builtin_amdgcn_s_memtime() : 0ull;
 #define NG_HAVE_LIN have_lin
+#define NG_WT_OUT kWtOut
 #include "ngicp_pass_group.inc"
+#undef NG_WT_OUT
 #undef NG_HAVE_LIN
 }
 #undef NG_STAMP
 
 template <int G, int WPS>
-__global__ void __launch_bounds__(256, WPS) k_gicp_pass_batch(BatchLaunch bl) {
+__global__ void __launch_bounds__(256, WPS) k_gicp_pass_batch(const PassArgs* records, BatchLaunch bl) {
   __shared__ WaveStage stage[4];
   __shared__ double lds[4][kNumSlots];
-  KernelBatchLaunch* kb = (KernelBatchLaunch*)__builtin_amdgcn_kernarg_segment_ptr();
+  KernelBatchLaunch* kb = batch_launch_args();
   const int lane_id = kb->lane[blockIdx.y];
-  KernelPassArgs* ka = (KernelPassArgs*)(unsigned long long)(reinterpret_cast<const PassArgs*>(kb->pass) + lane_id);
+  KernelPassArgs* ka = (KernelPassArgs*)(unsigned long long)(records + lane_id);
   typedef const int __attribute__((address_space(4))) * ConstIntPtr;
   const int done_now = ((KernelStatePtr)(unsigned long long)ka->st)->hot.done;
   const int order_is_valid = *(ConstIntPtr)(unsigned long long)ka->order_valid;
@@ -78,14 +89,14 @@
   batch_group_body<G, WPS>(*ka, group, stage, lds);
 }
 
-__global__ void __launch_bounds__(kSolveThreads) k_lm_solve_batch(BatchLaunch bl) {
+__global__ void __launch_bounds__(kSolveThreads) k_lm_solve_batch(const SolveArgs* records, BatchLaunch bl) {
   __shared__ SolveShared<kSolveThreads> sh;
-  KernelBatchLaunch* kb = (KernelBatchLaunch*)__builtin_amdgcn_kernarg_segment_ptr();
+  KernelBatchLaunch* kb = batch_launch_args();
   const int lane_id = kb->lane[blockIdx.x];
   static_assert(sizeof(SolveArgs) % 4 == 0, "SolveArgs is copied as dwords");
   constexpr int kWords = (int)(sizeof(SolveArgs) / 4);
   typedef const int __attribute__((address_space(4))) * ConstIntPtr;
-  ConstIntPtr src = (ConstIntPtr)(unsigned long long)(kb->solve + lane_id);
+  ConstIntPtr src = (ConstIntPtr)(unsigned long long)(records + lane_id);
   int w[kWords];
 #pragma unroll
   for (int i = 0; i < kWords; ++i) w[i] = src[i];
diff --git a/direct_lidar_odometry_amd/csrc/ngicp_lm.h b/direct_lidar_odometry_amd/csrc/ngicp_lm.h
--- a/direct_lidar_odometry_amd/csrc/ngicp_lm.h
+++ b/direct_lidar_odometry_amd/csrc/ngicp_lm.h
@@ -100,6 +100,18 @@
 
 static_assert(offsetof(SolveArgs, pass_ticks) == offsetof(SolveArgs, pass_honours_word) + 8, "serial_step takes no room of its own");
 
+template <int N>
+struct KernargPad {
+  unsigned char unused[N];
+};
+
+struct SolveHead {
+  LmState* st;
+  const double* partials;
+  const int* grp_cost;
+  int nblocks, nrows;
+};
+
 __host__ __device__ __forceinline__ int tri21(int r, int c) { return r * 6 - (r * (r - 1)) / 2 + (c - r); }
 
 constexpr int kMaxOrderGroups = 4096;
diff --git a/direct_lidar_odometry_amd/csrc/ngicp_pass.h b/direct_lidar_odometry_amd/csrc/ngicp_pass.h
--- a/direct_lidar_odometry_amd/csrc/ngicp_pass.h
+++ b/direct_lidar_odometry_amd/csrc/ngicp_pass.h
@@ -62,8 +62,10 @@
   } while (0)
 
 template <int G, int WPS = NGICP_PASS_WAVES, bool FUSED = false, bool ROBUST = false>
-__global__ void __launch_bounds__(256, WPS) k_gicp_pass(PassArgs a) {
+__global__ void __launch_bounds__(256, WPS) k_gicp_pass(const LmState* st_p, const int* order_valid_p, const int* grp_order_p, KernargPad<40> pad, PassArgs a) {
+  if constexpr (WPS < 4) asm volatile("" : "+s"(st_p), "+s"(order_valid_p), "+s"(grp_order_p));
   constexpr int B = 64 / G;
+  constexpr bool kWtOut = ((NGICP_PASS_WT_STORES >> (WPS >= 4 ? 1 : 0)) & 1) != 0;
   constexpr int kWin = WPS >= 4 ? 12 : 16, kSideStep = WPS >= 4 ? 8 : 16;
   static_assert(kWin <= kSortedPad, "walk windows may overhang the array by at most the sentinel frame");
   static_assert(B == kBatchQueries, "query batches are built for 32 queries (2 lanes per query)");
@@ -76,13 +78,13 @@
   __shared__ PassShared shm;
   __shared__ int last_block;
   WaveStage* stage_all = shm.stage;
-  const LmState* __restrict__ st = a.st;
+  const LmState* __restrict__ st = st_p;
   typedef const int __attribute__((address_space(4))) * ConstIntPtr;
   const int done_now = st->hot.done, have_lin_now = st->hot.have_lin;
   const int cur = st->hot.cur, nxt = cur ^ 1;
   const int lin_unneeded_now = st->hot.lin_unneeded;
-  const int order_is_valid = *(ConstIntPtr)(unsigned long long)a.order_valid;
-  const int order_entry = ((ConstIntPtr)(unsigned long long)a.grp_order)[blockIdx.x];
+  const int order_is_valid = *(ConstIntPtr)(unsigned long long)order_valid_p;
+  const int order_entry = ((ConstIntPtr)(unsigned long long)grp_order_p)[blockIdx.x];
   double R[9], t[3];
 #pragma unroll
   for (int i = 0; i < 9; ++i) R[i] = st->hot.xi.R[i];
@@ -174,7 +176,9 @@
   } else {
 #define NG_HAVE_LIN have_lin_now
 #define NG_ROBUST ROBUST
+#define NG_WT_OUT kWtOut
 #include "ngicp_pass_group.inc"
+#undef NG_WT_OUT
 #undef NG_ROBUST
 #undef NG_HAVE_LIN
   }
diff --git a/direct_lidar_odometry_amd/csrc/ngicp_pass_group.inc b/direct_lidar_odometry_amd/csrc/ngicp_pass_group.inc
--- a/direct_lidar_odometry_amd/csrc/ngicp_pass_group.inc
+++ b/direct_lidar_odometry_amd/csrc/ngicp_pass_group.inc
@@ -1,6 +1,10 @@
 #ifndef NG_ROBUST
 #define NG_ROBUST false
 #define NG_ROBUST_DEFAULTED
+#endif
+#ifndef NG_WT_OUT
+#define NG_WT_OUT false
+#define NG_WT_OUT_DEFAULTED
 #endif
   for (int item = group * 4 + wave; item < a.n_batches; item = a.n_batches) {
     typedef const int __attribute__((address_space(4))) * ConstBatchPtr;
@@ -409,7 +413,7 @@
       if (do_lin) {
         const int pos = mypos;
         const bool valid = (pos >= 0) && ((double)mybest < a.gate_sq);
-        if (!valid) tpt_new[i] = make_float4(0.f, 0.f, 0.f, __int_as_float(-1));
+        if (!valid) store_out16<NG_WT_OUT>(tpt_new + i, 0.f, 0.f, 0.f, __int_as_float(-1));
         if (valid) {
           ++nvalid;
           const double* CB = a.cov_tgt + (size_t)pos * 6;
@@ -418,7 +422,7 @@
           double ca[6];
 #pragma unroll
           for (int e = 0; e < 6; ++e) ca[e] = CA[e];
-          tpt_new[i] = make_float4(bp.x, bp.y, bp.z, __int_as_float(pos));
+          store_out16<NG_WT_OUT>(tpt_new + i, bp.x, bp.y, bp.z, __int_as_float(pos));
           double rcr[6], M[6];
           rotate_sym(R, ca, rcr);
 #pragma unroll
@@ -426,7 +430,7 @@
           inv3_sym(rcr, M);
           double* Mo = mahal_new + (size_t)i * 6;
 #pragma unroll
-          for (int e = 0; e < 6; ++e) Mo[e] = M[e];
+          for (int e = 0; e < 6; e += 2) store_out16<NG_WT_OUT>(Mo + e, M[e], M[e + 1]);
 
           const double ex = (double)bp.x - tax, ey = (double)bp.y - tay, ez = (double)bp.z - taz;
           if constexpr (NG_ROBUST) lin_terms_robust(acc, a.robust_kind, a.robust_c, a.robust_c2, tax, tay, taz, ex, ey, ez, M);
@@ -491,3 +495,7 @@
 #undef NG_ROBUST
 #undef NG_ROBUST_DEFAULTED
 #endif
+#ifdef NG_WT_OUT_DEFAULTED
+#undef NG_WT_OUT
+#undef NG_WT_OUT_DEFAULTED
+#endif
diff --git a/direct_lidar_odometry_amd/csrc/ngicp_search.h b/direct_lidar_odometry_amd/csrc/ngicp_search.h
--- a/direct_lidar_odometry_amd/csrc/ngicp_search.h
+++ b/direct_lidar_odometry_amd/csrc/ngicp_search.h
@@ -70,6 +70,30 @@
 #ifndef NGICP_ALIGNED_WINDOWS
 #define NGICP_ALIGNED_WINDOWS 0
 #endif
+#ifndef NGICP_PASS_WT_STORES
+#define NGICP_PASS_WT_STORES 0
+#endif
+template <bool WT>
+__device__ __forceinline__ void store_out16(float4* p, float x, float y, float z, float w) {
+  if constexpr (WT) {
+    typedef float V4f __attribute__((ext_vector_type(4)));
+    const V4f v = {x, y, z, w};
+    asm volatile("global_store_dwordx4 %0, %1, off sc1" ::"v"(p), "v"(v) : "memory");
+  } else {
+    *p = make_float4(x, y, z, w);
+  }
+}
+template <bool WT>
+__device__ __forceinline__ void store_out16(double* p, double x, double y) {
+  if constexpr (WT) {
+    typedef double V2d __attribute__((ext_vector_type(2)));
+    const V2d v = {x, y};
+    asm volatile("global_store_dwordx4 %0, %1, off sc1" ::"v"(p), "v"(v) : "memory");
+  } else {
+    p[0] = x;
+    p[1] = y;
+  }
+}
 constexpr int kWalkWindow = NGICP_WALK_WINDOW;
 static_assert(kWalkWindow <= kSortedPad && kWalkWindow % 2 == 0, "walk windows may overhang the array by at most the sentinel frame");
 
diff --git a/direct_lidar_odometry_amd/csrc/ngicp_solve.h b/direct_lidar_odometry_amd/csrc/ngicp_solve.h
--- a/direct_lidar_odometry_amd/csrc/ngicp_solve.h
+++ b/direct_lidar_odometry_amd/csrc/ngicp_solve.h
@@ -102,7 +102,7 @@
 }
 
 template <int THREADS, bool AGENT, bool PERSIST = false>
-__device__ __forceinline__ void lm_solve_body(const SolveArgs& a, SolveShared<THREADS>& sh) {
+__device__ __forceinline__ void lm_solve_body(const SolveArgs& a, SolveShared<THREADS>& sh, const SolveHead& hd) {
   static_assert(!PERSIST || AGENT, "the persistent solver is an agent-scope one");
   constexpr int kSolveThreads = THREADS;
   constexpr int kSolveSubs = 32;
@@ -116,8 +116,8 @@
   int& ord_arrived = sh.ord_arrived;
   LmHot& L = sh.L;
   if (threadIdx.x == 0) ord_arrived = 0;
-  LmState* st = a.st;
-  LmState* sto = a.st_out ? a.st_out : a.st;
+  LmState* st = hd.st;
+  LmState* sto = a.st_out ? a.st_out : hd.st;
 #define NG_SSTAMP(k)                                                                 \
   do {                                                                               \
     if (a.dbg_stamps && threadIdx.x == 0) a.dbg_stamps[k] = __builtin_amdgcn_s_memtime(); \
@@ -126,7 +126,7 @@
   const unsigned long long t_solver_entry = a.dbg_stamps ? __builtin_amdgcn_s_memtime() : 0ull;
   const int lane = threadIdx.x & 63, wave = threadIdx.x >> 6;
   const int vp = threadIdx.x & 15, sb = threadIdx.x >> 4;
-  const double2* __restrict__ rows = reinterpret_cast<const double2*>(a.partials) + vp;
+  const double2* __restrict__ rows = reinterpret_cast<const double2*>(hd.partials) + vp;
   static_assert(sizeof(LmHot) % 4 == 0, "LmHot is copied as dwords");
   constexpr int kHotWords = (int)(sizeof(LmHot) / 4), kHotPerThread = (kHotWords + kSolveThreads - 1) / kSolveThreads;
   constexpr int kCostPerThread = kMaxOrderGroups / kSolveThreads;
@@ -140,7 +140,7 @@
     if constexpr (PERSIST) hv[k] = w < kHotWords ? __hip_atomic_load(reinterpret_cast<const int*>(&st->hot) + w, __ATOMIC_RELAXED, __HIP_MEMORY_SCOPE_AGENT) : 0;
     else hv[k] = w < kHotWords ? reinterpret_cast<const int*>(&st->hot)[w] : 0;
   }
-  const int last_row = (a.nrows ? a.nrows : a.nblocks) - 1, last_grp = a.nblocks - 1;
+  const int last_row = (hd.nrows ? hd.nrows : hd.nblocks) - 1, last_grp = hd.nblocks - 1;
   auto load_row = [](const double2* q) -> double2 {
     if constexpr (PERSIST) {
       const double* d = reinterpret_cast<const double*>(q);
@@ -161,8 +161,8 @@
 #pragma unroll
   for (int k = 0; k < kCostPerThread; ++k) {
     const int gi = threadIdx.x + k * kSolveThreads;
-    if constexpr (PERSIST) oc[k] = (order_it && gi <= last_grp) ? __hip_atomic_load(a.grp_cost + gi, __ATOMIC_RELAXED, __HIP_MEMORY_SCOPE_AGENT) : 0;
-    else oc[k] = (order_it && gi <= last_grp) ? a.grp_cost[gi] : 0;
+    if constexpr (PERSIST) oc[k] = (order_it && gi <= last_grp) ? __hip_atomic_load(hd.grp_cost + gi, __ATOMIC_RELAXED, __HIP_MEMORY_SCOPE_AGENT) : 0;
+    else oc[k] = (order_it && gi <= last_grp) ? hd.grp_cost[gi] : 0;
   }
   double prior_v = 0.0;
   if (a.prior && threadIdx.x < kPriorDoubles) prior_v = a.prior[threadIdx.x];
@@ -321,9 +321,17 @@
 #undef NG_SSTAMP
 }
 
-__global__ void __launch_bounds__(kSolveThreads) k_lm_solve(SolveArgs a) {
+template <int THREADS, bool AGENT, bool PERSIST = false>
+__device__ __forceinline__ void lm_solve_body(const SolveArgs& a, SolveShared<THREADS>& sh) {
+  lm_solve_body<THREADS, AGENT, PERSIST>(a, sh, SolveHead{a.st, a.partials, a.grp_cost, a.nblocks, a.nrows});
+}
+
+__global__ void __launch_bounds__(kSolveThreads) k_lm_solve(LmState* st, const double* partials, const int* grp_cost, int nblocks, int nrows, KernargPad<32> pad, SolveArgs a) {
   __shared__ SolveShared<kSolveThreads> sh;
-  lm_solve_body<kSolveThreads, false>(a, sh);
+  lm_solve_body<kSolveThreads, false>(a, sh, SolveHead{st, partials, grp_cost, nblocks, nrows});
+}
+inline void launch_lm_solve(const SolveArgs& a, hipStream_t s) {
+  hipLaunchKernelGGL(k_lm_solve, dim3(1), dim3(kSolveThreads), 0, s, a.st, a.partials, a.grp_cost, a.nblocks, a.nrows, KernargPad<32>{}, a);
 }
 
 constexpr int kStepSelftestIn = 132;
diff --git a/direct_lidar_odometry_amd/csrc/ngicp_voxel.h b/direct_lidar_odometry_amd/csrc/ngicp_voxel.h
--- a/direct_lidar_odometry_amd/csrc/ngicp_voxel.h
+++ b/direct_lidar_odometry_amd/csrc/ngicp_voxel.h
@@ -310,8 +310,7 @@
 
 typedef const VoxelPassArgs __attribute__((address_space(4))) KernelVoxelPassArgs;
 
-__device__ __forceinline__ bool voxel_pass_begin(const VoxelPassArgs& a, PassPose& p) {
-  const LmState* __restrict__ st = a.st;
+__device__ __forceinline__ bool voxel_pass_begin(const LmState* __restrict__ st, const VoxelPassArgs& a, PassPose& p) {
   const int done_now = st->hot.done;
   load_pose(st, p);
   if (!(a.mode & 4) && done_now) return false;
@@ -320,10 +319,10 @@
 }
 
 template <bool ROBUST = false>
-__global__ void __launch_bounds__(kVoxBlock) k_vgicp_pass(VoxelPassArgs a) {
+__global__ void __launch_bounds__(kVoxBlock) k_vgicp_pass(const LmState* st, VoxelPassArgs a) {
   __shared__ VoxelPassLds sh;
   PassPose p;
-  if (!voxel_pass_begin(a, p)) return;
+  if (!voxel_pass_begin(st, a, p)) return;
   vgicp_pass_body<ROBUST>(a, p, sh);
 }
 
@@ -463,10 +462,10 @@
 }
 
 template <int K, bool ROBUST = false>
-__global__ void __launch_bounds__(kVoxBlock, 2) k_vgicp_pass_n(VoxelPassArgs a) {
+__global__ void __launch_bounds__(kVoxBlock, 2) k_vgicp_pass_n(const LmState* st, VoxelPassArgs a) {
   __shared__ VoxelPassLdsN<K> sh;
   PassPose p;
-  if (!voxel_pass_begin(a, p)) return;
+  if (!voxel_pass_begin(st, a, p)) return;
   vgicp_pass_n_body<K, ROBUST>(a, p, sh);
 }
 
diff --git a/direct_lidar_odometry_amd/csrc/ngicp_voxel_batch.h b/direct_lidar_odometry_amd/csrc/ngicp_voxel_batch.h
--- a/direct_lidar_odometry_amd/csrc/ngicp_voxel_batch.h
+++ b/direct_lidar_odometry_amd/csrc/ngicp_voxel_batch.h
@@ -14,12 +14,12 @@
 };
 
 template <int K>
-__global__ void __launch_bounds__(kVoxBlock, K == 1 ? 1 : 2) k_vgicp_pass_batch(BatchLaunch bl) {
+__global__ void __launch_bounds__(kVoxBlock, K == 1 ? 1 : 2) k_vgicp_pass_batch(const VoxelPassArgs* records, BatchLaunch bl) {
   static_assert(K == 1 || K == 7 || K == 27, "DIRECT1, DIRECT7 or DIRECT27");
   __shared__ typename VoxelBatchKernelTraits<K>::Lds sh;
-  KernelBatchLaunch* kb = (KernelBatchLaunch*)__builtin_amdgcn_kernarg_segment_ptr();
+  KernelBatchLaunch* kb = batch_launch_args();
   const int lane_id = kb->lane[blockIdx.y];
-  KernelVoxelPassArgs* ka = (KernelVoxelPassArgs*)(unsigned long long)(reinterpret_cast<const VoxelPassArgs*>(kb->pass) + lane_id);
+  KernelVoxelPassArgs* ka = (KernelVoxelPassArgs*)(unsigned long long)(records + lane_id);
   KernelStatePtr st4 = (KernelStatePtr)(unsigned long long)ka->st;
   if (st4->hot.done) return;
   PassPose p;
```

New measurement: 21180 (median of 6 runs). 1.6% higher.
